# calderpg/voxelized_geometry_tools

Hardware: AMD Instinct MI355X
Metric: Mvoxels/s for 1024^3 float SDF extract @1 GPU; % HBM roofline (higher is better)
Workload: dtype int32; 1 GPU; 1024^3 float SDF, D1 spheres seed 42, res 0.01, device-resident; workload_key=c4, parallelism=single GPU, edt_variant=0

## Files before the change

include/vgt_hip.h:

```cpp
#ifndef VGT_HIP_H_
#define VGT_HIP_H_

#include <stddef.h>
#include <stdint.h>

#ifdef __cplusplus
extern "C" {
#endif
#if defined(__GNUC__) || defined(__clang__)
#pragma GCC visibility push(default)
#endif

#define VGT_HIP_ABI_VERSION 2

typedef struct vgt_hip_ctx vgt_hip_ctx;
typedef struct vgt_hip_grids vgt_hip_grids;
typedef struct vgt_hip_filter vgt_hip_filter;

enum {
  VGT_HIP_OK = 0,
  VGT_HIP_ERR_INVALID_ARGUMENT = 1,
  VGT_HIP_ERR_RUNTIME = 2,
  VGT_HIP_ERR_UNAVAILABLE = 3
};
// ... 27 lines not shown
                               float max_range, const float* grid_pointcloud_transform,
                               float voxel_size, float inverse_voxel_size,
                               float grid_x_size, float grid_y_size, float grid_z_size,
                               int32_t num_x_voxels, int32_t num_y_voxels,
                               int32_t num_z_voxels);
int vgt_hip_raycast_pointcloud2_f32(vgt_hip_ctx* ctx, vgt_hip_grids* grids, size_t grid_index,
                                    const uint8_t* cloud_data_host, int64_t num_points,
                                    int64_t point_step, int64_t xyz_offset, float max_range,
                                    const float* grid_pointcloud_transform, float voxel_size,
                                    float inverse_voxel_size, float grid_x_size,
                                    float grid_y_size, float grid_z_size, int32_t num_x_voxels,
                                    int32_t num_y_voxels, int32_t num_z_voxels);
int vgt_hip_raycast_points_f32_dev(vgt_hip_ctx* ctx, vgt_hip_grids* grids, size_t grid_index,
                                   const float* points_xyz_dev, int64_t num_points,
                                   float max_range, const float* grid_pointcloud_transform,
                                   float voxel_size, float inverse_voxel_size,
                                   float grid_x_size, float grid_y_size, float grid_z_size,
                                   int32_t num_x_voxels, int32_t num_y_voxels,
                                   int32_t num_z_voxels);
int vgt_hip_raycast_points_f64(vgt_hip_ctx* ctx, vgt_hip_grids* grids, size_t grid_index,
                               const double* points_xyz_host, int64_t num_points,
                               double max_range, const double* grid_pointcloud_transform,
                               double voxel_size, double inverse_voxel_size,
                               double grid_x_size, double grid_y_size, double grid_z_size,
                               int32_t num_x_voxels, int32_t num_y_voxels,
                               int32_t num_z_voxels);

int vgt_hip_filter_grid_create(vgt_hip_ctx* ctx, int64_t num_cells,
                               const float* occupancy_host, vgt_hip_filter** out_filter);
int vgt_hip_filter_grid_create_deferred(vgt_hip_ctx* ctx, int64_t num_cells,
                                        const float* occupancy_host, vgt_hip_filter** out_filter);
void vgt_hip_filter_grid_destroy(vgt_hip_filter* filter);
int64_t vgt_hip_filter_grid_num_cells(const vgt_hip_filter* filter);
void* vgt_hip_filter_grid_dev_ptr(const vgt_hip_filter* filter);

int vgt_hip_filter_tracking_grids(vgt_hip_ctx* ctx, const vgt_hip_grids* grids,
                                  float percent_seen_free, int32_t outlier_points_threshold,
                                  int32_t num_cameras_seen_free, vgt_hip_filter* filter);
int vgt_hip_filter_tracking_grids_f64(vgt_hip_ctx* ctx, const vgt_hip_grids* grids,
                                      double percent_seen_free,
                                      int32_t outlier_points_threshold,
                                      int32_t num_cameras_seen_free, vgt_hip_filter* filter);

int vgt_hip_retrieve_tracking_grid(vgt_hip_ctx* ctx, const vgt_hip_grids* grids,
                                   size_t grid_index, void* host_out);
int vgt_hip_retrieve_filtered_grid(vgt_hip_ctx* ctx, const vgt_hip_filter* filter,
                                   void* host_out);


int vgt_hip_sdf_from_occupancy_f32(vgt_hip_ctx* ctx, const float* occupancy_host,
                                   int64_t nx, int64_t ny, int64_t nz, double resolution,
                                   int unknown_is_filled, int add_virtual_border,
                                   float* sdf_host, float* out_min, float* out_max);
int vgt_hip_sdf_from_mask_u8(vgt_hip_ctx* ctx, const uint8_t* filled_mask_host, int64_t nx,
                             int64_t ny, int64_t nz, double resolution,
                             int add_virtual_border, float* sdf_host, float* out_min,
                             float* out_max);

size_t vgt_hip_sdf_workspace_bytes(int64_t nx, int64_t ny, int64_t nz);
size_t vgt_hip_sdf_workspace_bytes_for_variant(int64_t nx, int64_t ny, int64_t nz, int variant);
int vgt_hip_sdf_dev(vgt_hip_ctx* ctx, const float* occupancy_dev, int64_t nx, int64_t ny,
                    int64_t nz, double resolution, int unknown_is_filled,
                    int add_virtual_border, float* sdf_dev, void* workspace_dev,
                    size_t workspace_bytes, float* minmax_dev);
int vgt_hip_sdf_dev_timed(vgt_hip_ctx* ctx, const float* occupancy_dev, int64_t nx,
                          int64_t ny, int64_t nz, double resolution, int unknown_is_filled,
                          int add_virtual_border, float* sdf_dev, void* workspace_dev,
                          size_t workspace_bytes, float* minmax_dev, float* kernel_ms);
size_t vgt_hip_sdf_batch_workspace_bytes(int64_t batch, int64_t nx, int64_t ny, int64_t nz);
int vgt_hip_sdf_batch_dev(vgt_hip_ctx* ctx, const float* occupancy_dev, int64_t batch, int64_t nx, int64_t ny,
                          int64_t nz, double resolution, int unknown_is_filled, int add_virtual_border,
                          float* sdf_dev, void* workspace_dev, size_t workspace_bytes, float* minmax_dev);
int vgt_hip_sdf_batch_from_occupancy_f32(vgt_hip_ctx* ctx, const float* const* occupancy_host, int64_t batch,
                                         int64_t nx, int64_t ny, int64_t nz, double resolution,
                                         int unknown_is_filled, int add_virtual_border, float* const* sdf_host,
                                         float* out_min, float* out_max);
#ifdef VGT_HIP_TESTING
int vgt_hip_set_edt_variant(vgt_hip_ctx* ctx, int variant);
int vgt_hip_debug_finalize_check(vgt_hip_ctx* ctx, int64_t first_d2, int64_t count,
                                 double resolution, uint64_t* mismatches,
                                 uint64_t* first_mismatch);
int vgt_hip_testing_set_host_pipeline_min_voxels(int64_t min_voxels);
int vgt_hip_testing_set_short_line_rows(int rows);
int vgt_hip_testing_set_check_spheres_workgroups(int workgroups);
int vgt_hip_testing_set_sphere_volume_workgroups(int workgroups);
int vgt_hip_testing_set_align_workgroups(int workgroups);
int vgt_hip_testing_set_kinematics_workgroups(int workgroups);
int vgt_hip_testing_set_motion_workgroups(int workgroups);
int vgt_hip_testing_set_cost_workgroups(int workgroups);
int vgt_hip_testing_motion_launch_geometry(int64_t num_links, int64_t num_spheres, int32_t* tile_samples,
                                           int32_t* table_in_lds);
int vgt_hip_testing_cost_launch_geometry(int64_t num_links, int64_t num_spheres, int gradient_form, int32_t* tile_samples,
                                         int32_t* passes, int32_t* table_in_lds, int32_t* links_in_lds);
int vgt_hip_testing_set_self_collision_workgroups(int workgroups);
int vgt_hip_testing_set_motion_self_workgroups(int workgroups);
int vgt_hip_testing_set_sphere_volume_counters(uint64_t* counters_dev);
size_t vgt_hip_testing_class_record_bytes(int64_t nx, int64_t ny, int64_t nz);
int vgt_hip_testing_class_records_dev(vgt_hip_ctx* ctx, const float* occupancy_dev, int64_t nx, int64_t ny, int64_t nz,
                                      int unknown_is_filled, int64_t z_offset, void* records_dev, void* summary_dev);
#endif

typedef struct vgt_hip_cells vgt_hip_cells;
int vgt_hip_cells_create(vgt_hip_ctx* ctx, const void* cells_host, int64_t nx, int64_t ny,
                         int64_t nz, int32_t cell_bytes, int32_t object_id_offset,
                         vgt_hip_cells** out_cells);
void vgt_hip_cells_destroy(vgt_hip_cells* cells);
int vgt_hip_cells_object_ids(vgt_hip_ctx* ctx, vgt_hip_cells* cells, uint32_t* ids_out,
                             int64_t capacity, int64_t* count);
int vgt_hip_cells_sdf(vgt_hip_ctx* ctx, vgt_hip_cells* cells, const uint32_t* objects_to_use,
                      int64_t num_objects, double resolution, int unknown_is_filled,
                      int add_virtual_border, float* sdf_host, float* out_min, float* out_max);
int vgt_hip_cells_object_sdfs(vgt_hip_ctx* ctx, vgt_hip_cells* cells, const uint32_t* object_ids,
                              int64_t num_objects, double resolution, int unknown_is_filled, int add_virtual_border,
                              float* const* sdf_host, float* out_min, float* out_max);
int vgt_hip_cells_free_and_named_objects_sdf(vgt_hip_ctx* ctx, vgt_hip_cells* cells,
                                             double resolution, int unknown_is_filled,
                                             int add_virtual_border, float* sdf_host,
                                             float* out_min, float* out_max);

int vgt_hip_timing_start(vgt_hip_ctx* ctx, int32_t max_calls);
int vgt_hip_timing_stop(vgt_hip_ctx* ctx, float* kernel_ms ,
                        int32_t* num_calls);

int vgt_hip_sdf_coarse_gradient(vgt_hip_ctx* ctx, const float* sdf_host, int64_t nx, int64_t ny,
                                int64_t nz, double resolution, int enable_edge_gradients,
                                const double* rotation, double* gradient_host,
                                uint8_t* has_value_host);
int vgt_hip_sdf_coarse_gradient_dev(vgt_hip_ctx* ctx, const float* sdf_dev, int64_t nx, int64_t ny,
                                    int64_t nz, double resolution, int enable_edge_gradients,
                                    const double* rotation, double* gradient_dev,
                                    uint8_t* has_value_dev);

int vgt_hip_sdf_estimate_distance(vgt_hip_ctx* ctx, const float* sdf_host, int64_t nx, int64_t ny, int64_t nz,
                                  double resolution, const double* grid_from_world, const double* query_xyz_host,
                                  int64_t num_queries, double* distance_host, uint8_t* has_value_host);
int vgt_hip_sdf_estimate_distance_dev(vgt_hip_ctx* ctx, const float* sdf_dev, int64_t nx, int64_t ny, int64_t nz,
                                      double resolution, const double* grid_from_world, const double* query_xyz_dev,
                                      int64_t num_queries, double* distance_dev, uint8_t* has_value_dev);
int vgt_hip_sdf_fine_gradient(vgt_hip_ctx* ctx, const float* sdf_host, int64_t nx, int64_t ny, int64_t nz,
                              double resolution, const double* grid_from_world, const double* query_xyz_host,
                              int64_t num_queries, double nominal_window_size, double* gradient_host,
                              uint8_t* has_value_host);

#define VGT_HIP_PROJECT_OK 0
#define VGT_HIP_PROJECT_OUTSIDE 1
#define VGT_HIP_PROJECT_FLAT_GRADIENT 2
#define VGT_HIP_PROJECT_LEFT_GRID 3
#define VGT_HIP_PROJECT_ITERATION_LIMIT 4
int vgt_hip_sdf_project_out_of_collision(vgt_hip_ctx* ctx, const float* sdf_host, int64_t nx, int64_t ny, int64_t nz,
                                         double resolution, const double* grid_from_world, const double* rotation,
                                         const double* query_xyz_host, int64_t num_queries, double minimum_distance,
                                         double stepsize_multiplier, int32_t max_iterations, double* position_host,
                                         uint8_t* has_value_host, uint8_t* status_host, int32_t* iterations_host);
int vgt_hip_sdf_project_out_of_collision_dev(vgt_hip_ctx* ctx, const float* sdf_dev, int64_t nx, int64_t ny, int64_t nz,
                                             double resolution, const double* grid_from_world, const double* rotation,
                                             const double* query_xyz_dev, int64_t num_queries, double minimum_distance,
                                             double stepsize_multiplier, int32_t max_iterations, double* position_dev,
                                             uint8_t* has_value_dev, uint8_t* status_dev, int32_t* iterations_dev);

#define VGT_HIP_SEGMENT_OCCUPANCY 0
#define VGT_HIP_SEGMENT_SDF_BELOW 1
#define VGT_HIP_SEGMENT_WALK_THROUGH 1u
#define VGT_HIP_SEGMENT_CLEAR 0
#define VGT_HIP_SEGMENT_HIT 1
#define VGT_HIP_SEGMENT_MISSED_GRID 2
#define VGT_HIP_SEGMENT_INVALID 3
// ... 414 lines not shown
```

voxelized_geometry_tools_amd/capi.py:

```python
import collections
import ctypes
import threading
import weakref
import os

import numpy as np

_HERE = os.path.dirname(os.path.abspath(__file__))
LIB_PATH = os.environ.get("VGT_HIP_LIB") or os.path.join(_HERE, "libvgt_hip.so")
TESTING_LIB_PATH = os.environ.get("VGT_HIP_TESTING_LIB") or os.path.join(_HERE, "libvgt_hip_testing.so")
_LIB = None

_i64 = ctypes.c_int64
_i32 = ctypes.c_int32
_f32 = ctypes.c_float
_f64 = ctypes.c_double
_p = ctypes.c_void_p
_sz = ctypes.c_size_t
_int = ctypes.c_int

SIGNATURES = {
    "vgt_hip_abi_version": (_int, []),
    "vgt_hip_last_error": (ctypes.c_char_p, []),
    "vgt_hip_device_count": (_int, [ctypes.POINTER(_int)]),
# ... 104 lines not shown
    "vgt_hip_check_motions_with_self_dev": (_int, [_p, _p, _i64, _i64, _i64, _f64, _p, _p, _p, _p, _i64, _p, _i64, _p, _p,
                                                   _p, _p, _i32, _i64, _p, _p, _f64, _f64, ctypes.c_uint32, _p, _p, _p,
                                                   _p, _p, _p, _p, _p, _p, _p, _p]),
    "vgt_hip_motion_self_tile_samples": (_i32, [_i64, _i64]),
    "vgt_hip_nearest_workspace_bytes": (ctypes.c_size_t, [_i64, _i64, _i64]),
    "vgt_hip_nearest_dev": (_int, [_p, _p, _i64, _i64, _i64, _int, _p, _p, _p, ctypes.c_size_t]),
    "vgt_hip_nearest_from_occupancy_f32": (_int, [_p, _p, _i64, _i64, _i64, _int, _p, _p]),
    "vgt_hip_nearest_from_mask_u8": (_int, [_p, _p, _i64, _i64, _i64, _p, _p]),
    "vgt_hip_cells_nearest": (_int, [_p, _p, _p, _i64, _int, _p, _p, _p]),
    "vgt_hip_sdf_local_extrema_map": (_int, [_p, _p, _i64, _i64, _i64, _f64, _p, _p]),
    "vgt_hip_sdf_local_extrema_map_dev": (_int, [_p, _p, _i64, _i64, _i64, _f64, _p, _p]),
    "vgt_hip_connected_components": (_int, [_p, _p, _i64, _i64, _i64, _p, _p]),
    "vgt_hip_connected_components_dev": (_int, [_p, _p, _i64, _i64, _i64, _p, _p]),
    "vgt_hip_cells_connected_components": (_int, [_p, _p, _int, _p, _p]),
    "vgt_hip_cells_spatial_segments": (_int, [_p, _p, _p, _f64, _p, _p]),
    "vgt_hip_cells_spatial_segments_dev": (_int, [_p, _p, _p, _f64, _p, _p]),
    "vgt_hip_cells_update_spatial_segments": (_int, [_p, _p, _f64, _f64, _int, _int, _p, _p, _p]),
    "vgt_hip_component_surface_mask": (_int, [_p, _p, _p, _i64, _i64, _i64, _int, _p]),
    "vgt_hip_component_surface_mask_dev": (_int, [_p, _p, _p, _i64, _i64, _i64, _int, _p]),
    "vgt_hip_select_cells": (_int, [_p, _p, _p, _i64, _i64, _i64, _int, _int, _f32, _p, _p, _p, _i64, _p]),
    "vgt_hip_select_cells_dev": (_int, [_p, _p, _p, _i64, _i64, _i64, _int, _int, _f32, _p, _p, _p, _i64, _p]),
    "vgt_hip_cells_select": (_int, [_p, _p, _p, _int, _int, _p, _p, _p, _int, _i64, _p]),
    "vgt_hip_extract_surface": (_int, [_p, _p, _i64, _i64, _i64, _f32, _int, _f64, _p, _p, _p, _i64, _p, _i64, _p, _p]),
    "vgt_hip_extract_surface_dev": (_int, [_p, _p, _i64, _i64, _i64, _f32, _int, _f64, _p, _p, _p, _i64, _p, _i64, _p,
                                           _p]),
    "vgt_hip_cells_extract_surface": (_int, [_p, _p, _f64, _p, _p, _p, _i64, _p, _i64, _p, _p]),
    "vgt_hip_travel_cost_workspace_bytes": (ctypes.c_size_t, [_i64, _i64, _i64]),
    "vgt_hip_travel_cost": (_int, [_p, _p, _i64, _i64, _i64, _i32, _int, _f64, _p, ctypes.c_uint32, _p, _p, _i64,
                                   ctypes.c_uint32, _p, _p, _p]),
    "vgt_hip_travel_cost_dev": (_int, [_p, _p, _i64, _i64, _i64, _i32, _int, _f64, _p, ctypes.c_uint32, _p, _p, _i64,
                                       ctypes.c_uint32, _p, _p, _p, _p, _sz]),
    "vgt_hip_cells_travel_cost": (_int, [_p, _p, _p, _i64, _int, _p, ctypes.c_uint32, _p, _p, _i64, ctypes.c_uint32, _p,
                                         _p, _p]),
    "vgt_hip_trace_paths": (_int, [_p, _p, _i64, _p, _i64, _i32, _p, _p, _p]),
    "vgt_hip_trace_paths_dev": (_int, [_p, _p, _i64, _p, _i64, _i32, _p, _p, _p]),
    "vgt_hip_component_topology_dev": (_int, [_p, _p, _p, _i64, _i64, _i64, _int, ctypes.c_uint32, _p]),
    "vgt_hip_component_topology": (_int, [_p, _p, _i64, _i64, _i64, _int, _p, _p, _p, ctypes.c_uint64]),
    "vgt_hip_cells_component_topology": (_int, [_p, _p, _int, _int, _p, _p, _p, ctypes.c_uint64]),
    "vgt_hip_rasterize_mesh": (_int, [_p, _p, _i64, _p, _i64, _p, _int, _i64, _i64, _i64, _f64, _p, _p, _int, _int]),
    "vgt_hip_rasterize_mesh_dev": (_int, [_p, _p, _i64, _p, _i64, _p, _int, _i64, _i64, _i64, _f64, _p, _p, _int, _int]),
    "vgt_hip_mesh_grid_for": (_int, [_p, _i64, _f64, _p, _p, _p, _p]),
    "vgt_hip_fill_enclosed": (_int, [_p, _p, _int, _i64, _i64, _i64, _int, _p]),
    "vgt_hip_fill_enclosed_dev": (_int, [_p, _p, _int, _i64, _i64, _i64, _int, _p]),
    "vgt_hipx_sdf_multi": (_int, [_p, _int, _p, _i64, _i64, _i64, _f64, _int, _int, _p, _p, _p]),
    "vgt_hipx_release": (None, []),
    "vgt_hipx_last_timing": (_int, [_p]),
    "vgt_hipx_point_share": (_int, [_i64, _i32, _i32, _p, _p]),
    "vgt_hipx_raycast_points_split": (_int, [_p, _p, _sz, _p, _int, _p, _i64, _f32, _p, _f32, _f32, _f32, _f32,
                                             _f32, _i32, _i32, _i32]),
    "vgt_hip_sdf_dev": (_int, [_p, _p, _i64, _i64, _i64, _f64, _int, _int, _p, _p, _sz, _p]),
    "vgt_hip_sdf_dev_timed": (_int, [_p, _p, _i64, _i64, _i64, _f64, _int, _int, _p, _p, _sz, _p, _p]),
    "vgt_hip_sdf_batch_workspace_bytes": (_sz, [_i64, _i64, _i64, _i64]),
    "vgt_hip_sdf_batch_dev": (_int, [_p, _p, _i64, _i64, _i64, _i64, _f64, _int, _int, _p, _p, _sz, _p]),
    "vgt_hip_sdf_batch_from_occupancy_f32": (_int, [_p, _p, _i64, _i64, _i64, _i64, _f64, _int, _int, _p, _p, _p]),
    "vgt_hip_cells_object_sdfs": (_int, [_p, _p, _p, _i64, _f64, _int, _int, _p, _p, _p]),
    "vgt_hip_cells_create": (_int, [_p, _p, ctypes.c_int64, ctypes.c_int64, ctypes.c_int64, ctypes.c_int32,
                                   ctypes.c_int32, _p]),
    "vgt_hip_cells_destroy": (None, [_p]),
    "vgt_hip_cells_object_ids": (_int, [_p, _p, _p, ctypes.c_int64, _p]),
    "vgt_hip_cells_sdf": (_int, [_p, _p, _p, ctypes.c_int64, ctypes.c_double, _int, _int, _p, _p, _p]),
    "vgt_hip_cells_free_and_named_objects_sdf": (_int, [_p, _p, ctypes.c_double, _int, _int, _p, _p, _p]),
    "vgt_hip_sdf_coarse_gradient": (_int, [_p, _p, ctypes.c_int64, ctypes.c_int64, ctypes.c_int64, ctypes.c_double,
                                          _int, _p, _p, _p]),
    "vgt_hip_sdf_coarse_gradient_dev": (_int, [_p, _p, ctypes.c_int64, ctypes.c_int64, ctypes.c_int64,
                                              ctypes.c_double, _int, _p, _p, _p]),
    "vgt_hip_sdf_slab_carries_dev": (_int, [_p, _p, ctypes.c_int32, ctypes.c_int32, ctypes.c_int64, ctypes.c_int64,
                                            ctypes.c_int64, _p]),
    "vgt_hip_timing_start": (_int, [_p, ctypes.c_int32]),
    "vgt_hip_timing_stop": (_int, [_p, _p, _p]),
    "vgt_hip_sdf_slab_summary_bytes": (_sz, [_i64, _i64]),
    "vgt_hip_sdf_slab_carries_bytes": (_sz, [_i64, _i64]),
    "vgt_hip_sdf_slab_range": (_int, [_i64, ctypes.c_int32, ctypes.c_int32, _p, _p]),
    "vgt_hip_sdf_slab_begin_dev": (_int, [_p, _p, _i64, _i64, _i64, _i64, _int, _p, _sz, _p, _p]),
    "vgt_hip_sdf_slab_finish_dev": (_int, [_p, _i64, _i64, _i64, _i64, _i64, _f64, _int, _p, _p, _p,
                                           _sz, _p, _p]),
}


TESTING_SIGNATURES = {
    "vgt_hip_set_edt_variant": (_int, [_p, _int]),
    "vgt_hip_debug_finalize_check": (_int, [_p, ctypes.c_int64, ctypes.c_int64, ctypes.c_double, _p, _p]),
    "vgt_hip_testing_set_host_pipeline_min_voxels": (_int, [ctypes.c_int64]),
    "vgt_hip_testing_set_short_line_rows": (_int, [_int]),
    "vgt_hip_testing_set_check_spheres_workgroups": (_int, [_int]),
    "vgt_hip_testing_set_sphere_volume_workgroups": (_int, [_int]),
    "vgt_hip_testing_set_align_workgroups": (_int, [_int]),
    "vgt_hip_testing_set_kinematics_workgroups": (_int, [_int]),
    "vgt_hip_testing_set_motion_workgroups": (_int, [_int]),
    "vgt_hip_testing_set_cost_workgroups": (_int, [_int]),
    "vgt_hip_testing_motion_launch_geometry": (_int, [_i64, _i64, _p, _p]),
    "vgt_hip_testing_cost_launch_geometry": (_int, [_i64, _i64, _int, _p, _p, _p, _p]),
    "vgt_hip_testing_set_self_collision_workgroups": (_int, [_int]),
    "vgt_hip_testing_set_motion_self_workgroups": (_int, [_int]),
    "vgt_hip_testing_set_sphere_volume_counters": (_int, [_p]),
    "vgt_hip_testing_class_record_bytes": (_sz, [_i64, _i64, _i64]),
    "vgt_hip_testing_class_records_dev": (_int, [_p, _p, _i64, _i64, _i64, _int, _i64, _p, _p]),
}


MESH_RULE_REFERENCE = 0
MESH_RULE_NEAREST = 1

PROJECT_OK = 0
PROJECT_OUTSIDE = 1
PROJECT_FLAT_GRADIENT = 2
PROJECT_LEFT_GRID = 3
PROJECT_ITERATION_LIMIT = 4

SEGMENT_OCCUPANCY = 0
SEGMENT_SDF_BELOW = 1
SEGMENT_WALK_THROUGH = 1
SEGMENT_CLEAR = 0
SEGMENT_HIT = 1
SEGMENT_MISSED_GRID = 2
SEGMENT_INVALID = 3

SPHERES_OUTSIDE_IS_COLLISION = 1
SPHERES_CLEAR = 0
SPHERES_COLLISION = 1
SPHERES_NO_VALUE = 2
SPHERES_KEEP = 1
JOINT_FIXED, JOINT_REVOLUTE, JOINT_PRISMATIC = 0, 1, 2
FK_NOT_COMPUTABLE = 1
FK_OUTSIDE_LIMITS = 2
IK_CONVERGED = 0
IK_ITERATION_LIMIT = 1
IK_DEGENERATE = 2
IK_NOT_COMPUTABLE = 3
MOTION_STOP_AT_COLLISION = 2
MOTION_CLEAR = 0
MOTION_COLLISION = 1
MOTION_NO_VALUE = 2
MOTION_INVALID = 3
SELF_NO_VALUE_IS_COLLISION = 1
SELF_CLEAR = 0
SELF_COLLISION = 1
SELF_NO_VALUE = 2
SELF_PAIRS_SKIP_ADJACENT = 1
MOTION_SELF_NO_VALUE_IS_COLLISION = 4
MOTION_CAUSE_ENVIRONMENT = 1
MOTION_CAUSE_SELF = 2
ALIGN_CONVERGED = 0
ALIGN_ITERATION_LIMIT = 1
ALIGN_DEGENERATE = 2
ALIGN_TOO_FEW = 3

SELECT_ALL = 0
SELECT_SURFACE_26 = 1
SELECT_COMPONENT_SURFACE = 2
CLASS_ABOVE = 0x01
CLASS_BELOW = 0x02
CLASS_EQUAL = 0x04
CLASS_UNORDERED = 0x08
CELL_MEMBER_NONE = 0
CELL_MEMBER_OBJECT_ID = 1
CELL_MEMBER_COMPONENT = 2
CELL_MEMBER_SPATIAL_SEGMENT = 3

COMPONENT_TOPOLOGY = np.dtype([(name, np.int32) for name in (
    "present", "num_holes", "num_voids", "num_surfaces", "m3", "m5", "m6", "num_surface_vertices")])


SegmentCasts = collections.namedtuple("SegmentCasts", "status hit_index hit_fraction cells_examined min_value min_index")


SphereChecks = collections.namedtuple(
# ... 1030 lines not shown
        if not isinstance(cells, np.ndarray) or cells.ndim != 3 or not cells.flags.c_contiguous or \
                not cells.flags.writeable:
            raise ValueError("cells must be a writeable C-contiguous (nx, ny, nz) array")
        count = _i64(0)
        check(self._lib.vgt_hip_fill_enclosed(self.handle, _ptr(cells), cells.dtype.itemsize, *cells.shape,
                                              int(bool(unknown_is_filled)), ctypes.byref(count)))
        return int(count.value)

    def fill_enclosed_dev(self, cells_ptr, cell_bytes, shape, unknown_is_filled=True, want_count=True):
        count = _i64(0)
        check(self._lib.vgt_hip_fill_enclosed_dev(self.handle, _ptr(cells_ptr), int(cell_bytes),
                                                  *[int(c) for c in shape], int(bool(unknown_is_filled)),
                                                  ctypes.byref(count) if want_count else None))
        return int(count.value) if want_count else None

    def mesh_sdf(self, vertices, triangles, resolution, rule=MESH_RULE_REFERENCE, unknown_is_filled=True,
                 add_virtual_border=False, with_occupancy=False, solid=False):
        import torch
        v = np.ascontiguousarray(vertices, dtype=np.float64).reshape(-1, 3)
        t = np.ascontiguousarray(triangles, dtype=np.int32).reshape(-1, 3)
        shape, origin = mesh_grid_for(v, resolution)
        wfg = np.eye(4)
        wfg[:3, 3] = origin
        gfw = np.eye(4)
        gfw[:3, 3] = -origin
        device = "cuda:%d" % self._lib.vgt_hip_device_of(self.handle)
        v_dev = torch.from_numpy(v).to(device)
        t_dev = torch.from_numpy(t).to(device)
        occ_dev = torch.zeros(shape, dtype=torch.float32, device=device)
        sdf_dev = torch.empty(shape, dtype=torch.float32, device=device)
        ws_bytes = sdf_workspace_bytes(shape)
        ws_dev = torch.empty(ws_bytes, dtype=torch.uint8, device=device)
        minmax_dev = torch.empty(2, dtype=torch.float32, device=device)
        torch.cuda.synchronize(device)
        self.rasterize_mesh_dev(v_dev.data_ptr(), len(v), t_dev.data_ptr(), len(t), occ_dev.data_ptr(), 4, shape,
                                resolution, wfg.T.reshape(16), gfw.T.reshape(16), True, rule)
        if solid:
            self.fill_enclosed_dev(occ_dev.data_ptr(), 4, shape, unknown_is_filled, want_count=False)
        self.sdf_dev(occ_dev.data_ptr(), shape, resolution, sdf_dev.data_ptr(), ws_dev.data_ptr(), ws_bytes,
                     minmax_dev.data_ptr(), unknown_is_filled, add_virtual_border)
        self.synchronize()
        lo, hi = (float(x) for x in minmax_dev.cpu().numpy())
        out = (sdf_dev.cpu().numpy(), lo, hi, origin)
        return out + (occ_dev.cpu().numpy(),) if with_occupancy else out

    def trim(self):
        check(self._lib.vgt_hip_trim(self.handle))

    def set_stream(self, stream_ptr):
        check(self._lib.vgt_hip_set_stream(self.handle, _ptr(stream_ptr) if stream_ptr else None))

    def reset_stream(self):
        check(self._lib.vgt_hip_reset_stream(self.handle))

    def synchronize(self):
        check(self._lib.vgt_hip_synchronize(self.handle))

    def timing_start(self, max_calls):
        self._timing_capacity = int(max_calls)
        check(self._lib.vgt_hip_timing_start(self.handle, int(max_calls)))

    def timing_stop(self):
        out = np.zeros((self._timing_capacity, 3), dtype=np.float32)
        n = ctypes.c_int32(0)
        check(self._lib.vgt_hip_timing_stop(self.handle, _ptr(out), ctypes.byref(n)))
        return out[:n.value].copy()

    def set_edt_variant(self, variant):
        if not self.testing:
            if int(variant) == 0:
                return
            raise VgtHipError("EDT variants other than 0 exist in libvgt_hip_testing.so only: Context(testing=True)")
        check(self._lib.vgt_hip_set_edt_variant(self.handle, int(variant)))

    def class_records(self, occ_ptr, shape, unknown_is_filled=True, z_offset=0, records_ptr=None, summary_ptr=None):
        nx, ny, nz = shape
        check(self._lib.vgt_hip_testing_class_records_dev(self.handle, _ptr(occ_ptr), nx, ny, nz,
                                                          int(bool(unknown_is_filled)), int(z_offset), _ptr(records_ptr),
                                                          _ptr(summary_ptr)))

    def set_short_line_rows(self, rows):
        check(self._lib.vgt_hip_testing_set_short_line_rows(int(rows)))

    def set_check_spheres_workgroups(self, workgroups):
        check(self._lib.vgt_hip_testing_set_check_spheres_workgroups(int(workgroups)))

    def set_sphere_volume_workgroups(self, workgroups):
        check(self._lib.vgt_hip_testing_set_sphere_volume_workgroups(int(workgroups)))

    def set_align_workgroups(self, workgroups):
        check(self._lib.vgt_hip_testing_set_align_workgroups(int(workgroups)))

    def set_kinematics_workgroups(self, workgroups):
        check(self._lib.vgt_hip_testing_set_kinematics_workgroups(int(workgroups)))

    def set_motion_workgroups(self, workgroups):
        check(self._lib.vgt_hip_testing_set_motion_workgroups(int(workgroups)))

    def set_cost_workgroups(self, workgroups):
        check(self._lib.vgt_hip_testing_set_cost_workgroups(int(workgroups)))

    def set_self_collision_workgroups(self, workgroups):
        check(self._lib.vgt_hip_testing_set_self_collision_workgroups(int(workgroups)))

    def set_motion_self_workgroups(self, workgroups):
        check(self._lib.vgt_hip_testing_set_motion_self_workgroups(int(workgroups)))

    def set_sphere_volume_counters(self, counters_ptr):
        check(self._lib.vgt_hip_testing_set_sphere_volume_counters(_ptr(counters_ptr)))

    def set_host_pipeline_min_voxels(self, min_voxels):
        check(self._lib.vgt_hip_testing_set_host_pipeline_min_voxels(int(min_voxels)))

    def debug_finalize_check(self, first_d2, count, resolution):
        bad = ctypes.c_uint64(0)
        first = ctypes.c_uint64(0)
        check(self._lib.vgt_hip_debug_finalize_check(self.handle, int(first_d2), int(count), float(resolution),
                                                     ctypes.byref(bad), ctypes.byref(first)))
        return int(bad.value), (None if first.value == 2 ** 64 - 1 else int(first.value))

    def sdf_coarse_gradient(self, sdf, resolution, enable_edge_gradients=False, rotation=None):
        field = np.ascontiguousarray(sdf, dtype=np.float32)
        nx, ny, nz = field.shape
        grad = np.empty((nx, ny, nz, 3), dtype=np.float64)
        has = np.empty((nx, ny, nz), dtype=np.uint8)
        rot = None if rotation is None else np.ascontiguousarray(rotation, dtype=np.float64).reshape(9)
        check(self._lib.vgt_hip_sdf_coarse_gradient(self.handle, _ptr(field), nx, ny, nz, float(resolution),
                                                    int(bool(enable_edge_gradients)), _ptr(rot), _ptr(grad),
                                                    _ptr(has)))
        return grad, has.astype(bool)

    def cells(self, records, shape, object_id_offset=4):
        return Cells(self, records, shape, object_id_offset)

    def sdf_from_occupancy(self, occupancy, resolution, unknown_is_filled=True,
                           add_virtual_border=False, out=None):
        occ = np.ascontiguousarray(occupancy, dtype=np.float32)
        if occ.ndim != 3:
            raise ValueError("occupancy must be (nx, ny, nz)")
        nx, ny, nz = occ.shape
        if out is None:
            out = np.empty(occ.shape, dtype=np.float32)
        elif out.shape != occ.shape or out.dtype != np.float32 or not out.flags.c_contiguous:
            raise ValueError("out must be a C-contiguous float32 array of the occupancy's shape")
        lo, hi = _f32(), _f32()
        check(self._lib.vgt_hip_sdf_from_occupancy_f32(
            self.handle, _ptr(occ), nx, ny, nz, float(resolution), int(bool(unknown_is_filled)),
            int(bool(add_virtual_border)), _ptr(out), ctypes.byref(lo), ctypes.byref(hi)))
        return out, lo.value, hi.value

    def sdf_batch_from_occupancy(self, grids, resolution, unknown_is_filled=True, add_virtual_border=False):
        grids = [np.ascontiguousarray(g, dtype=np.float32) for g in grids]
        if not grids or any(g.ndim != 3 or g.shape != grids[0].shape for g in grids):
            raise ValueError("a batch is a non-empty list of (nx, ny, nz) grids of one shape")
        nx, ny, nz = grids[0].shape
        outs = [np.empty(g.shape, dtype=np.float32) for g in grids]
        batch = len(grids)
        in_ptrs = (ctypes.c_void_p * batch)(*[g.ctypes.data for g in grids])
        out_ptrs = (ctypes.c_void_p * batch)(*[o.ctypes.data for o in outs])
        lo = np.zeros(batch, dtype=np.float32)
        hi = np.zeros(batch, dtype=np.float32)
        check(self._lib.vgt_hip_sdf_batch_from_occupancy_f32(
            self.handle, ctypes.cast(in_ptrs, ctypes.c_void_p), batch, nx, ny, nz, float(resolution),
            int(bool(unknown_is_filled)), int(bool(add_virtual_border)), ctypes.cast(out_ptrs, ctypes.c_void_p),
            _ptr(lo), _ptr(hi)))
        return outs, lo, hi
# ... 567 lines not shown
```

voxelized_geometry_tools_amd/csrc/edt_kernels.hip:

```cpp
#include "edt_device.hpp"

namespace vgt
{
namespace
{
__global__ __launch_bounds__(256) void SlabCarriesKernel(const SlabLineSummary* __restrict__ summaries,
                                                        int world, int rank, int64_t lines, int nz_global,
                                                        SlabLineCarry* __restrict__ carries)
{
  const int share = nz_global / world, extra = nz_global % world;
  for (int64_t line = static_cast<int64_t>(blockIdx.x) * blockDim.x + threadIdx.x; line < lines;
       line += static_cast<int64_t>(gridDim.x) * blockDim.x)
  {
    int prev_filled = -1, prev_free = -1, next_filled = -1, next_free = -1;
    for (int r = 0; r < rank; r++)
    {
      const uint16_t rec = summaries[static_cast<int64_t>(r) * lines + line].last;
      const int end = (r + 1) * share + min(r + 1, extra) - 1;
      const int other = (rec & kSlabNone) == kSlabNone ? -1 : static_cast<int>(rec & kSlabNone);
      const bool filled = (rec & kSlabFilledBit) != 0;
      prev_filled = max(prev_filled, filled ? end : other);
      prev_free = max(prev_free, filled ? other : end);
    }
    for (int r = world - 1; r > rank; r--)
    {
      const uint16_t rec = summaries[static_cast<int64_t>(r) * lines + line].first;
      const int begin = r * share + min(r, extra);
      const int other = (rec & kSlabNone) == kSlabNone ? -1 : static_cast<int>(rec & kSlabNone);
      const bool filled = (rec & kSlabFilledBit) != 0;
      const int first_filled = filled ? begin : other, first_free = filled ? other : begin;
      if (first_filled >= 0) next_filled = first_filled;
      if (first_free >= 0) next_free = first_free;
    }
    SlabLineCarry c;
    c.prev_filled = static_cast<int16_t>(prev_filled);
    c.next_filled = static_cast<int16_t>(next_filled);
    c.prev_free = static_cast<int16_t>(prev_free);
    c.next_free = static_cast<int16_t>(next_free);
    carries[line] = c;
  }
}

__global__ void InitMinMaxKernel(uint32_t* minmax_enc, int count)
{
  for (int i = static_cast<int>(threadIdx.x); i < count; i += static_cast<int>(blockDim.x))
  {
    minmax_enc[2 * i] = 0xffffffffu;
    minmax_enc[2 * i + 1] = 0u;
  }
}
__global__ void DecodeMinMaxKernel(const uint32_t* minmax_enc, float* out, int count)
{
  for (int i = static_cast<int>(threadIdx.x); i < 2 * count; i += static_cast<int>(blockDim.x))
    out[i] = DecodeOrdered(minmax_enc[i]);
}

int GridFor(int64_t work_items, int block)
{
  const int64_t blocks = (work_items + block - 1) / block;
  const int64_t cap = 256 * 32;
  return static_cast<int>(blocks < 1 ? 1 : (blocks > cap ? cap : blocks));
}
}

hipError_t LaunchSlabCarries(const SlabLineSummary* summaries, int world, int rank, int64_t lines, int64_t nz_global,
                             SlabLineCarry* carries, hipStream_t stream)
{
  hipLaunchKernelGGL(SlabCarriesKernel, dim3(GridFor(lines, 256)), dim3(256), 0, stream, summaries, world, rank,
                     lines, static_cast<int>(nz_global), carries);
  return hipGetLastError();
}

hipError_t LaunchPassXFinalize(const int32_t* in32, float* sdf, uint32_t* minmax_enc, SweepScratch scratch,
                               const SdfParams& p, hipStream_t stream)
{
  return LaunchPassXFinalizeRange(in32, sdf, minmax_enc, scratch, p, 0, -1, stream);
}

hipError_t LaunchPassXFinalizeRange(const int32_t* in32, float* sdf, uint32_t* minmax_enc, SweepScratch scratch,
                                    const SdfParams& p, int64_t outer_begin, int64_t outer_count, hipStream_t stream)
{
  if (p.nx <= ShortLineRows())
    return LaunchPassXShortFinalizeRange(in32, sdf, minmax_enc, p, outer_begin, outer_count, stream);
  return LaunchPassXSweepFinalizeRange(in32, sdf, minmax_enc, scratch, p, outer_begin, outer_count, stream);
}

hipError_t LaunchInitMinMax(uint32_t* minmax_enc, hipStream_t stream, int64_t count)
{
  hipLaunchKernelGGL(InitMinMaxKernel, dim3(1), dim3(count > 1 ? 64 : 1), 0, stream, minmax_enc, static_cast<int>(count));
  return hipGetLastError();
}

hipError_t LaunchDecodeMinMax(const uint32_t* minmax_enc, float* minmax_out, hipStream_t stream, int64_t count)
{
  hipLaunchKernelGGL(DecodeMinMaxKernel, dim3(1), dim3(count > 1 ? 64 : 1), 0, stream, minmax_enc, minmax_out,
                     static_cast<int>(count));
  return hipGetLastError();
}
}
```

voxelized_geometry_tools_amd/csrc/edt_line_geom.hpp:

```cpp
#pragma once

#include "vgt_internal.hpp"

namespace vgt
{
struct SweepGeom
{
  int n;
  int nz;
  int zsegs;
  int items;
  int outers;
  int groups;
  int nwords;
  int chunks;
  int64_t row_stride;
  int64_t outer_stride;
  int nx, ny;
  int pass_axis;
  double resolution;
  int add_virtual_border;
  int z_offset, nz_global;
  int outer_begin;
  int batch_outers;
  int64_t batch_skip;
};

inline SweepGeom SweepGeometry(const SdfParams& p, int axis, int64_t* outer_count)
{
  SweepGeom g{};
  g.nz = static_cast<int>(p.nz);
  g.nx = static_cast<int>(p.nx);
  g.ny = static_cast<int>(p.ny);
  g.pass_axis = axis;
  if (axis == 0)
  {
    g.n = static_cast<int>(p.nx);
    g.row_stride = p.ny * p.nz;
    g.outer_stride = p.nz;
    *outer_count = p.ny;
  }
  else
  {
    g.n = static_cast<int>(p.ny);
    g.row_stride = p.nz;
    g.outer_stride = p.ny * p.nz;
    *outer_count = p.nx;
  }
  g.resolution = p.resolution;
  g.add_virtual_border = p.add_virtual_border;
  g.z_offset = static_cast<int>(p.z_offset);
  g.nz_global = static_cast<int>(p.nz_global > 0 ? p.nz_global : p.nz);
  return g;
}
}
```

voxelized_geometry_tools_amd/csrc/edt_record_kernels.hip:

```cpp
#include "edt_device.hpp"

#ifndef VGT_REC_EXP
#define VGT_REC_EXP 0
#endif
namespace vgt
{
namespace
{
constexpr int kRecordBlock = 256;
constexpr int kRecordWaves = kRecordBlock / kWaveSize;
constexpr int kNoTransitionBelow = -(1 << 20);
constexpr int kNoTransitionAbove = 1 << 20;

template <bool kUnknownFilled>
__device__ __forceinline__ bool IsFilledCell(float occupancy)
{
  return kUnknownFilled ? (occupancy >= 0.5f) : (occupancy > 0.5f);
}
template <bool kUnknownFilled>
__device__ __forceinline__ bool IsFilledCell(uint8_t mask)
{
  return mask != 0;
}

__device__ __forceinline__ void WriteLane(uint32_t& value, uint32_t word_uniform, int target)
{
  asm("s_nop 3\n\tv_writelane_b32 %0, %1, %2" : "+v"(value) : "s"(word_uniform), "n"(target));
}

__device__ __forceinline__ uint32_t EncodeBelow(int t, int word_begin)
{
  return (t == kNoTransitionBelow) ? kRecordNoneBelow : static_cast<uint32_t>(2 * (t - word_begin)) + kRecordBias;
}
__device__ __forceinline__ uint32_t EncodeAbove(int t, int word_begin)
{
  return (t == kNoTransitionAbove) ? kRecordNoneAbove : static_cast<uint32_t>(2 * (t - word_begin)) + kRecordBias;
}

__device__ __forceinline__ uint16_t SummaryField(bool filled, int other_local, int z_offset)
{
  return static_cast<uint16_t>((filled ? kSlabFilledBit : 0u) |
                               (other_local < 0 ? kSlabNone : static_cast<uint16_t>(other_local + z_offset)));
}

template <typename InT, int W, bool kUnknownFilled>
__global__ __launch_bounds__(kRecordBlock) void ClassRecordKernel(const InT* __restrict__ in,
                                                                 ClassRecord* __restrict__ records,
                                                                 int64_t num_lines, int ny, int nz, int nwords,
                                                                 SlabLineSummary* __restrict__ summary, int z_offset,
                                                                 int mark_no_site)
{
  constexpr int L = kWaveSize / W;
  const int lane = threadIdx.x & (kWaveSize - 1);
  const int wave = __builtin_amdgcn_readfirstlane(static_cast<int>(threadIdx.x) / kWaveSize);
  const int j = lane / W, w = lane % W;
  const int64_t num_steps = (num_lines + L - 1) / L;
  for (int64_t step = static_cast<int64_t>(blockIdx.x) * kRecordWaves + wave; step < num_steps;
       step += static_cast<int64_t>(gridDim.x) * kRecordWaves)
  {
    const int64_t line0 = step * L;
    const int lines_here = static_cast<int>(min(static_cast<int64_t>(L), num_lines - line0));
    InT v[L][W];
#pragma unroll
    for (int jj = 0; jj < L; jj++)
    {
      const InT* line_in = in + (line0 + min(jj, lines_here - 1)) * nz;
#pragma unroll
      for (int c = 0; c < W; c++)
      {
        const int z = min(min(c, nwords - 1) * kWaveSize + lane, nz - 1);
#if VGT_REC_EXP & 2
        v[jj][c] = line_in[z];
#else
        v[jj][c] = __builtin_nontemporal_load(line_in + z);
#endif
      }
    }
    uint32_t mlo = 0, mhi = 0;
#pragma unroll
    for (int jj = 0; jj < L; jj++)
    {
#pragma unroll
      for (int c = 0; c < W; c++)
      {
        const uint64_t m = __builtin_amdgcn_ballot_w64(IsFilledCell<kUnknownFilled>(v[jj][c]));
        WriteLane(mlo, static_cast<uint32_t>(m), jj * W + c);
        WriteLane(mhi, static_cast<uint32_t>(m >> 32), jj * W + c);
      }
    }
    const bool valid = j < lines_here && w < nwords;
    const uint64_t m = (static_cast<uint64_t>(mhi) << 32) | mlo;
    const uint32_t next_bit0 = static_cast<uint32_t>(__shfl_down(static_cast<int>(mlo & 1u), 1, W));
    const bool boundary = valid && (w + 1 < nwords) && (((mhi >> 31) & 1u) != next_bit0);
    const uint64_t inner = (m ^ (m >> 1)) & 0x7fffffffffffffffull;
    const uint64_t transitions = valid ? (inner | (boundary ? 0x8000000000000000ull : 0ull)) : 0ull;
    const int word_begin = w * kWaveSize;
    int last_t = kNoTransitionBelow, first_t = kNoTransitionAbove;
    if (transitions)
    {
      last_t = word_begin + 63 - __clzll(static_cast<long long>(transitions));
      first_t = word_begin + __ffsll(static_cast<long long>(transitions)) - 1;
    }
    int upto = last_t;
    int from = first_t;
#pragma unroll
    for (int d = 1; d < W; d *= 2)
    {
      const int a = __shfl_up(upto, d, W);
      const int b = __shfl_down(from, d, W);
      if (w >= d) upto = max(upto, a);
      if (w + d < W) from = min(from, b);
    }
    int below = __shfl_up(upto, 1, W);
    if (w == 0) below = kNoTransitionBelow;
    int above = __shfl_down(from, 1, W);
    if (w == W - 1) above = kNoTransitionAbove;
    if (boundary) above = word_begin + 63;
    const int line_last = __shfl(upto, W - 1, W);
    const int line_first = __shfl(from, 0, W);
    if (valid)
    {
      const uint32_t line = static_cast<uint32_t>(line0) + static_cast<uint32_t>(j);
      const int64_t x = line / static_cast<uint32_t>(ny);
      const int y = static_cast<int>(line - static_cast<uint32_t>(x) * static_cast<uint32_t>(ny));
      ClassRecord r;
      r.mask_lo = mlo;
      r.mask_hi = mhi;
      r.below2 = EncodeBelow(below, word_begin);
      r.above2 = EncodeAbove(above, word_begin);
      if (mark_no_site && line_last == kNoTransitionBelow) r.above2 = kRecordNoSite;
      using Raw = uint32_t __attribute__((ext_vector_type(4)));
      Raw raw;
      raw.x = r.mask_lo;
      raw.y = r.mask_hi;
      raw.z = r.below2;
      raw.w = r.above2;
#if VGT_REC_EXP & 1
      if (raw.x == 0x12345u)
#endif
      *reinterpret_cast<Raw*>(records + ((x * nwords + w) * ny + y)) = raw;
    }
    if (summary)
    {
      const uint32_t first_class = static_cast<uint32_t>(__shfl(static_cast<int>(mlo & 1u), 0, W));
      const int last_word = nwords - 1;
      const int last_bit = (nz - 1) & 63;
      const uint32_t my_last = static_cast<uint32_t>((m >> last_bit) & 1ull);
      const uint32_t last_class = static_cast<uint32_t>(__shfl(static_cast<int>(my_last), last_word, W));
      if (j < lines_here && w == 0)
      {
        SlabLineSummary s;
        s.first = SummaryField(first_class != 0u, line_first == kNoTransitionAbove ? -1 : line_first + 1, z_offset);
        s.last = SummaryField(last_class != 0u, line_last == kNoTransitionBelow ? -1 : line_last, z_offset);
        summary[line0 + j] = s;
      }
    }
  }
}

template <typename InT, bool kUnknownFilled>
__global__ __launch_bounds__(kRecordBlock) void ClassRecordLongLineKernel(const InT* __restrict__ in,
                                                                         ClassRecord* __restrict__ records,
                                                                         int64_t num_lines, int ny, int nz, int nwords,
                                                                         SlabLineSummary* __restrict__ summary,
                                                                         int z_offset, int mark_no_site)
{
  constexpr int kMaxWords = static_cast<int>(kMaxExtent / kWaveSize);
  __shared__ uint64_t s_mask[kRecordWaves][kMaxWords];
  __shared__ int32_t s_below[kRecordWaves][kMaxWords];
  __shared__ int32_t s_above[kRecordWaves][kMaxWords];
  __shared__ int32_t s_line[kRecordWaves][2];
  const int lane = threadIdx.x & (kWaveSize - 1);
  const int wave = threadIdx.x / kWaveSize;
  volatile uint64_t* mask = s_mask[wave];
  volatile int32_t* below = s_below[wave];
  volatile int32_t* above = s_above[wave];
  volatile int32_t* ends = s_line[wave];
  for (int64_t line = static_cast<int64_t>(blockIdx.x) * kRecordWaves + wave; line < num_lines;
       line += static_cast<int64_t>(gridDim.x) * kRecordWaves)
  {
    for (int c = 0; c < nwords; c++)
    {
      const int z = min(c * kWaveSize + lane, nz - 1);
      const uint64_t m = __builtin_amdgcn_ballot_w64(IsFilledCell<kUnknownFilled>(in[line * nz + z]));
      if (lane == 0) mask[c] = m;
    }
    __builtin_amdgcn_wave_barrier();
    if (lane == 0)
    {
      int last = kNoTransitionBelow;
      for (int c = 0; c < nwords; c++)
      {
        below[c] = last;
        const uint64_t m = mask[c];
        uint64_t t = (m ^ (m >> 1)) & 0x7fffffffffffffffull;
        if (c + 1 < nwords && ((m >> 63) & 1ull) != (mask[c + 1] & 1ull)) t |= 0x8000000000000000ull;
        if (t) last = c * kWaveSize + 63 - __clzll(static_cast<long long>(t));
      }
      ends[1] = last;
      int first = kNoTransitionAbove;
      for (int c = nwords - 1; c >= 0; c--)
      {
        const uint64_t m = mask[c];
        const bool boundary = c + 1 < nwords && ((m >> 63) & 1ull) != (mask[c + 1] & 1ull);
        above[c] = boundary ? c * kWaveSize + 63 : first;
        uint64_t t = (m ^ (m >> 1)) & 0x7fffffffffffffffull;
        if (boundary) t |= 0x8000000000000000ull;
        if (t) first = c * kWaveSize + __ffsll(static_cast<long long>(t)) - 1;
      }
      ends[0] = first;
    }
    __builtin_amdgcn_wave_barrier();
    const int64_t x = line / ny;
    const int y = static_cast<int>(line - x * ny);
    const int line_first = ends[0], line_last = ends[1];
    for (int c = lane; c < nwords; c += kWaveSize)
    {
      const uint64_t m = mask[c];
      ClassRecord r;
      r.mask_lo = static_cast<uint32_t>(m);
      r.mask_hi = static_cast<uint32_t>(m >> 32);
      r.below2 = EncodeBelow(below[c], c * kWaveSize);
      r.above2 = EncodeAbove(above[c], c * kWaveSize);
      if (mark_no_site && line_last == kNoTransitionBelow) r.above2 = kRecordNoSite;
      records[(x * nwords + c) * ny + y] = r;
    }
    if (summary && lane == 0)
    {
      const bool first_class = (mask[0] & 1ull) != 0ull;
      const bool last_class = ((mask[nwords - 1] >> ((nz - 1) & 63)) & 1ull) != 0ull;
      SlabLineSummary s;
      s.first = SummaryField(first_class, line_first == kNoTransitionAbove ? -1 : line_first + 1, z_offset);
      s.last = SummaryField(last_class, line_last == kNoTransitionBelow ? -1 : line_last, z_offset);
      summary[line] = s;
    }
    __builtin_amdgcn_wave_barrier();
  }
}

__global__ __launch_bounds__(256) void SlabRecordFixupKernel(ClassRecord* __restrict__ records,
                                                            const SlabLineCarry* __restrict__ carries, int64_t nx,
                                                            int ny, int nwords, int z_offset)
{
  const int64_t total = nx * nwords * static_cast<int64_t>(ny);
  for (int64_t i = static_cast<int64_t>(blockIdx.x) * blockDim.x + threadIdx.x; i < total;
       i += static_cast<int64_t>(gridDim.x) * blockDim.x)
  {
    ClassRecord r = records[i];
    const bool none_below = r.below2 == kRecordNoneBelow, none_above = r.above2 == kRecordNoneAbove;
    if (!none_below && !none_above) continue;
    const int y = static_cast<int>(i % ny);
    const int64_t xw = i / ny;
    const int w = static_cast<int>(xw % nwords);
    const int64_t x = xw / nwords;
    const SlabLineCarry c = carries[x * ny + y];
    const int word_begin = w * kWaveSize;
    bool changed = false;
    if (none_below)
    {
      const bool filled = (r.mask_lo & 1u) != 0u;
      const int other = filled ? c.prev_free : c.prev_filled;
      if (other >= 0)
      {
        r.below2 = EncodeBelow(other - z_offset, word_begin);
        changed = true;
      }
    }
    if (none_above)
    {
      const bool filled = (r.mask_hi >> 31) != 0u;
      const int other = filled ? c.next_free : c.next_filled;
      if (other >= 0)
      {
        r.above2 = EncodeAbove(other - 1 - z_offset, word_begin);
        changed = true;
      }
    }
    const uint64_t m = (static_cast<uint64_t>(r.mask_hi) << 32) | r.mask_lo;
    const bool uniform = (m ^ (m >> 1)) << 1 == 0ull;
    if (r.below2 == kRecordNoneBelow && r.above2 == kRecordNoneAbove && uniform)
    {
      r.above2 = kRecordNoSite;
      changed = true;
    }
    if (changed) records[i] = r;
  }
}

int RecordGridFor(int64_t steps)
{
  const int64_t blocks = (steps + kRecordWaves - 1) / kRecordWaves;
  const int64_t cap = 256 * 32;
  return static_cast<int>(blocks < 1 ? 1 : (blocks > cap ? cap : blocks));
}

template <typename InT, bool kUnknownFilled>
hipError_t LaunchRecords(const InT* in, ClassRecord* records, const SdfParams& p, SlabLineSummary* summary,
                         hipStream_t stream)
{
  const int64_t lines = p.nx * p.ny;
  const int nz = static_cast<int>(p.nz), ny = static_cast<int>(p.ny);
  const int nwords = static_cast<int>(RecordWords(p.nz));
  const int z_offset = static_cast<int>(p.z_offset);
  const int mark_no_site = summary == nullptr ? 1 : 0;
#define VGT_RECORD_CASE(W)                                                                                          \
  hipLaunchKernelGGL((ClassRecordKernel<InT, W, kUnknownFilled>), dim3(RecordGridFor((lines + 64 / W - 1) / (64 / W))), \
                     dim3(kRecordBlock), 0, stream, in, records, lines, ny, nz, nwords, summary, z_offset,          \
                     mark_no_site)
  if (nwords <= 1)
    VGT_RECORD_CASE(1);
  else if (nwords <= 2)
    VGT_RECORD_CASE(2);
  else if (nwords <= 4)
    VGT_RECORD_CASE(4);
  else if (nwords <= 8)
    VGT_RECORD_CASE(8);
  else if (nwords <= 16)
    VGT_RECORD_CASE(16);
  else if (nwords <= 32)
    VGT_RECORD_CASE(32);
  else if (nwords <= 64)
    VGT_RECORD_CASE(64);
  else
    hipLaunchKernelGGL((ClassRecordLongLineKernel<InT, kUnknownFilled>), dim3(RecordGridFor(lines)), dim3(kRecordBlock),
                       0, stream, in, records, lines, ny, nz, nwords, summary, z_offset, mark_no_site);
#undef VGT_RECORD_CASE
  return hipGetLastError();
}
}

hipError_t LaunchClassRecordsFromOccupancy(const float* occupancy, ClassRecord* records, const SdfParams& p,
                                           SlabLineSummary* summary, hipStream_t stream)
{
  if (p.unknown_is_filled) return LaunchRecords<float, true>(occupancy, records, p, summary, stream);
  return LaunchRecords<float, false>(occupancy, records, p, summary, stream);
}

hipError_t LaunchClassRecordsFromMask(const uint8_t* mask, ClassRecord* records, const SdfParams& p,
                                      SlabLineSummary* summary, hipStream_t stream)
{
  return LaunchRecords<uint8_t, false>(mask, records, p, summary, stream);
}

hipError_t LaunchSlabRecordFixup(ClassRecord* records, const SlabLineCarry* carries, const SdfParams& p,
                                 hipStream_t stream)
{
  const int nwords = static_cast<int>(RecordWords(p.nz));
  const int64_t total = p.nx * nwords * p.ny;
  const int64_t blocks = (total + 255) / 256;
  const int grid = static_cast<int>(blocks < 1 ? 1 : (blocks > 256 * 32 ? 256 * 32 : blocks));
  hipLaunchKernelGGL(SlabRecordFixupKernel, dim3(grid), dim3(256), 0, stream, records, carries, p.nx,
                     static_cast<int>(p.ny), nwords, static_cast<int>(p.z_offset));
  return hipGetLastError();
}
}
```

voxelized_geometry_tools_amd/csrc/edt_sweep_kernels.hip:

```cpp
#include "edt_device.hpp"
#include "edt_line_geom.hpp"

#include <cstdlib>
#include <type_traits>

namespace vgt
{
namespace
{
#ifndef VGT_SWEEP_BAND
#define VGT_SWEEP_BAND 16
#endif
#ifndef VGT_SWEEP_RING
#define VGT_SWEEP_RING 32
#endif
#ifndef VGT_SWEEP_CHUNK
#define VGT_SWEEP_CHUNK 8
#endif
#ifndef VGT_SWEEP_WAVES
#define VGT_SWEEP_WAVES 4
#endif
#ifndef VGT_SWEEP_GROUP
#define VGT_SWEEP_GROUP 2
#endif
constexpr int kBand = VGT_SWEEP_BAND;
constexpr int kWord = 32;
#ifndef VGT_SWEEP_INFO_BLOCK
#define VGT_SWEEP_INFO_BLOCK 2
#endif
constexpr int kInfoBlock = VGT_SWEEP_INFO_BLOCK;
static_assert(kInfoBlock >= 1, "sizes");
#ifndef VGT_SWEEP_RING_WIDE
#define VGT_SWEEP_RING_WIDE 16
#endif
#ifndef VGT_SWEEP_CHUNK_WIDE
#define VGT_SWEEP_CHUNK_WIDE 4
#endif
#ifndef VGT_SWEEP_GROUPS
#define VGT_SWEEP_GROUPS 8
#endif
constexpr int kSweepGroups = VGT_SWEEP_GROUPS;
constexpr int kCounterStride = 32;
constexpr int kMaxSweepSlots = 4096;
template <bool kPacked>
struct RingShape
{
  static constexpr int kRing = kPacked ? VGT_SWEEP_RING : VGT_SWEEP_RING_WIDE;
  static constexpr int kChunk = kPacked ? VGT_SWEEP_CHUNK : VGT_SWEEP_CHUNK_WIDE;
  static_assert(kBand % kChunk == 0 && kRing >= 4 * kChunk && (kRing & (kRing - 1)) == 0 && kChunk % 4 == 0, "sizes");
};
constexpr int kFar = 32768;
static_assert(kWord % kBand == 0 && kBand % 2 == 0, "sizes");
#ifdef VGT_HOST_EMULATION
uint64_t class_band_tally[3] = {0, 0, 0};
uint64_t ring_checks = 0, ring_spills = 0;
constexpr uint32_t kInfoPoison = 0xdeadbeefu;
uint64_t sign_word_reads = 0;
#endif


template <bool kPacked>
struct Codec;
template <>
struct Codec<true>
{
  using Entry = uint32_t;
  static constexpr int32_t kSentinelG = (1 << 22) - 3;
  static __device__ __forceinline__ Entry Pack(int32_t G, int row)
  {
    return (static_cast<uint32_t>(G) << 10) | static_cast<uint32_t>(row);
  }
  static __device__ __forceinline__ int32_t G(Entry e) { return static_cast<int32_t>(e >> 10); }
  static __device__ __forceinline__ int Row(Entry e) { return static_cast<int>(e & 1023u); }
  static __device__ __forceinline__ Entry Unknown() { return ~0u; }
  static __device__ __forceinline__ bool IsUnknown(Entry e) { return e == ~0u; }
};
template <>
struct Codec<false>
{
  using Entry = uint2;
  static constexpr int32_t kSentinelG = 1 << 30;
  static __device__ __forceinline__ Entry Pack(int32_t G, int row)
  {
    return make_uint2(static_cast<uint32_t>(G), static_cast<uint32_t>(row));
  }
  static __device__ __forceinline__ int32_t G(Entry e) { return static_cast<int32_t>(e.x); }
  static __device__ __forceinline__ int Row(Entry e) { return static_cast<int>(e.y); }
  static __device__ __forceinline__ Entry Unknown() { return make_uint2(0u, ~0u); }
  static __device__ __forceinline__ bool IsUnknown(Entry e) { return e.y == ~0u; }
};

#ifndef VGT_SWEEP_NT
#define VGT_SWEEP_NT 3
#endif
__device__ __forceinline__ void StoreQuad(uint4* p, uint32_t a, uint32_t b, uint32_t c, uint32_t d)
{
#if defined(VGT_HOST_EMULATION) || !(VGT_SWEEP_NT & 8)
  *p = make_uint4(a, b, c, d);
#else
  using Raw = uint32_t __attribute__((ext_vector_type(4)));
  Raw r;
  r.x = a; r.y = b; r.z = c; r.w = d;
  __builtin_nontemporal_store(r, reinterpret_cast<Raw*>(p));
#endif
}
__device__ __forceinline__ uint4 LoadQuad(const uint4* p)
{
#if defined(VGT_HOST_EMULATION) || !(VGT_SWEEP_NT & 8)
  return *p;
#else
  using Raw = uint32_t __attribute__((ext_vector_type(4)));
  const Raw r = __builtin_nontemporal_load(reinterpret_cast<const Raw*>(p));
  return make_uint4(r.x, r.y, r.z, r.w);
#endif
}
__device__ __forceinline__ void StorePair(uint2* p, uint32_t a, uint32_t b)
{
#if defined(VGT_HOST_EMULATION) || !(VGT_SWEEP_NT & 4)
  *p = make_uint2(a, b);
#else
  using Raw = uint32_t __attribute__((ext_vector_type(2)));
  Raw r;
  r.x = a; r.y = b;
  __builtin_nontemporal_store(r, reinterpret_cast<Raw*>(p));
#endif
}
__device__ __forceinline__ uint2 LoadPair(const uint2* p)
{
#if defined(VGT_HOST_EMULATION) || !(VGT_SWEEP_NT & 4)
  return *p;
#else
  using Raw = uint32_t __attribute__((ext_vector_type(2)));
  const Raw r = __builtin_nontemporal_load(reinterpret_cast<const Raw*>(p));
  return make_uint2(r.x, r.y);
#endif
}

template <int N>
__device__ __forceinline__ void StoreChunk(uint32_t* dst, const uint32_t (&e)[N])
{
// ... 109 lines not shown
__device__ __forceinline__ uint32_t AbsDiffPlusOne(uint32_t a, uint32_t b_uniform)
{
  return (max(a, b_uniform) - min(a, b_uniform)) + 1u;
}
__device__ __forceinline__ uint32_t SpreadLaneMask(uint64_t mask_uniform, [[maybe_unused]] int lane)
{
#ifdef VGT_HOST_EMULATION
  return ((mask_uniform >> lane) & 1ull) ? ~0u : 0u;
#else
  return __builtin_amdgcn_inverse_ballot_w64(mask_uniform) ? ~0u : 0u;
#endif
}

__device__ __forceinline__ void TakeLoaded([[maybe_unused]] uint32_t& v)
{
#ifndef VGT_HOST_EMULATION
  asm volatile("" : "+v"(v));
#endif
}
__device__ __forceinline__ void TakeLoaded(uint4& v)
{
  TakeLoaded(v.x);
  TakeLoaded(v.y);
  TakeLoaded(v.z);
  TakeLoaded(v.w);
}

__device__ __forceinline__ uint32_t LowBits(int bits)
{
  return (bits >= 32) ? ~0u : ((1u << bits) - 1u);
}

#if defined(VGT_HOST_EMULATION) || !(VGT_SWEEP_NT & 1)
#define VGT_STREAM_LOAD(p) (*(p))
#else
#define VGT_STREAM_LOAD(p) __builtin_nontemporal_load(p)
#endif
#if defined(VGT_HOST_EMULATION) || !(VGT_SWEEP_NT & 2)
#define VGT_STREAM_STORE(v, p) (*(p) = (v))
#else
#define VGT_STREAM_STORE(v, p) __builtin_nontemporal_store(v, p)
#endif

#ifdef VGT_HOST_EMULATION
#define VGT_COLD_PATH()
#define VGT_MIN_F32(acc, v) acc = fminf(acc, v)
#define VGT_MAX_F32(acc, v) acc = fmaxf(acc, v)
#define VGT_MIN3_F32(acc, a, b) acc = fminf(acc, fminf(a, b))
#define VGT_MAX3_F32(acc, a, b) acc = fmaxf(acc, fmaxf(a, b))
#else
#define VGT_COLD_PATH() asm volatile("; rare path")
#define VGT_MIN_F32(acc, v) asm("v_min_f32 %0, %0, %1" : "+v"(acc) : "v"(v))
#define VGT_MAX_F32(acc, v) asm("v_max_f32 %0, %0, %1" : "+v"(acc) : "v"(v))
#define VGT_MIN3_F32(acc, a, b) asm("v_min3_f32 %0, %0, %1, %2" : "+v"(acc) : "v"(a), "v"(b))
#define VGT_MAX3_F32(acc, a, b) asm("v_max3_f32 %0, %0, %1, %2" : "+v"(acc) : "v"(a), "v"(b))
#endif


__device__ __forceinline__ void WaveMinMax(float lo_value, float hi_value, uint32_t* minmax_enc)
{
  uint32_t lo = 0xffffffffu, hi = 0u;
  if (lo_value <= hi_value)
  {
    lo = EncodeOrdered(lo_value);
    hi = EncodeOrdered(hi_value);
  }
#ifdef VGT_HOST_EMULATION
  minmax_enc[0] = min(minmax_enc[0], lo);
  minmax_enc[1] = max(minmax_enc[1], hi);
#else
  for (int off = kWaveSize / 2; off > 0; off >>= 1)
  {
    lo = min(lo, static_cast<uint32_t>(__shfl_xor(static_cast<int>(lo), off)));
    hi = max(hi, static_cast<uint32_t>(__shfl_xor(static_cast<int>(hi), off)));
  }
  if (threadIdx.x == 0)
  {
    atomicMin(&minmax_enc[0], lo);
    atomicMax(&minmax_enc[1], hi);
  }
#endif
}

template <typename InT, typename OutT, bool kFinal, bool kPacked, bool kPlain>
__global__ __launch_bounds__(kWaveSize, VGT_SWEEP_WAVES) void SweepPassKernel(const InT* __restrict__ in,
                                                                            OutT* __restrict__ out,
                                                                            unsigned char* __restrict__ spill,
                                                                            uint2* __restrict__ word_info,
                                                                            uint32_t* __restrict__ minmax_enc,
                                                                            int* __restrict__ work_counter,
                                                                            const SweepGeom g)
{
  using C = Codec<kPacked>;
  using Entry = typename C::Entry;
  constexpr bool kRecords = std::is_same<InT, ClassRecord>::value;
  constexpr bool kSignBlocks = !kFinal;
  constexpr bool kTakeSignWords = !kSignBlocks;
  static_assert(!(kRecords && kFinal), "records feed the Y pass");
  constexpr int kRing = RingShape<kPacked>::kRing;
  constexpr int kChunk = RingShape<kPacked>::kChunk;
  constexpr int32_t kLimit = C::kSentinelG;
  constexpr int kEntryBytes = static_cast<int>(sizeof(Entry));
  constexpr int kShift = kPacked ? 8 : 9;
  constexpr uint32_t kSlot = 1u << kShift;
  constexpr uint32_t kRingMask = (kRing - 1) << kShift;
  constexpr int kChunkBytes = kChunk * kEntryBytes;
  constexpr uint32_t kChunkSlots = static_cast<uint32_t>(kChunk) << kShift;
  __shared__ Entry ring[kRing * kWaveSize];
  unsigned char* const ring_bytes = reinterpret_cast<unsigned char*>(ring);

  const int lane = threadIdx.x;
  const int n = g.n;
  const int64_t rstride = g.row_stride;
  unsigned char* const own_spill = spill + static_cast<int64_t>(blockIdx.x) * g.chunks * (kWaveSize * kChunkBytes);
  uint2* const own_info = word_info + static_cast<int64_t>(blockIdx.x) * (g.nwords + 1) * kWaveSize;
  const uint32_t lane_entry = static_cast<uint32_t>(lane) * kEntryBytes;
  const uint32_t lane_chunk = static_cast<uint32_t>(lane) * kChunkBytes;
  float lo_value = INFINITY, hi_value = -INFINITY;
  constexpr bool kUseTable = kFinal && kPlain && kPacked && (1024 / kBand <= 64);
  constexpr uint32_t kSmallD2 = 512;
  [[maybe_unused]] float* small_table = nullptr;
  if constexpr (kUseTable)
  {
    __shared__ float small_table_storage[kSmallD2];
    small_table = small_table_storage;
#ifdef VGT_HOST_EMULATION
    for (uint32_t d2 = 0; d2 < kSmallD2; d2++)
#else
    for (uint32_t d2 = static_cast<uint32_t>(lane); d2 < kSmallD2; d2 += kWaveSize)
#endif
      small_table[d2] = SqrtTimesResolutionExact(static_cast<int32_t>(d2), g.resolution);
    __syncthreads();
  }
#ifdef VGT_HOST_EMULATION
  int emulated_round = 0;
#endif
  [[maybe_unused]] auto fetch_item = [&]() -> int {
    int fetched = 0;
#ifndef VGT_HOST_EMULATION
    const int group = static_cast<int>(blockIdx.x) % g.groups;
    if (lane == 0) fetched = atomicAdd(work_counter + group * kCounterStride, 1);
    fetched = __builtin_amdgcn_readfirstlane(fetched);
    const int dealt = fetched / g.zsegs;
    fetched = (dealt * g.groups + group) * g.zsegs + (fetched - dealt * g.zsegs);
#endif
    return fetched;
  };
  for (;;)
  {
  int item = 0;
  unsigned char* wave_spill = own_spill;
  uint2* wave_info = own_info;
#ifdef VGT_HOST_EMULATION
  item = static_cast<int>(blockIdx.x + gridDim.x * emulated_round++);
#else
  item = fetch_item();
#endif
  if (item >= g.items) break;
#ifdef VGT_HOST_EMULATION
  for (int64_t w = 0; w < g.nwords + 1; w++) wave_info[w * kWaveSize + lane] = make_uint2(kInfoPoison, kInfoPoison);
#endif
  const int outer = item / g.zsegs;
  const int z0 = (item - outer * g.zsegs) * kWaveSize;
  const bool batched = g.batch_outers != g.outers;
  const int batch_index = batched ? outer / g.batch_outers : 0;
  const int outer_in_grid = outer - batch_index * g.batch_outers;
  const int64_t outer_offset = static_cast<int64_t>(outer) * g.outer_stride + static_cast<int64_t>(batch_index) * g.batch_skip;
  const uint32_t zl = static_cast<uint32_t>(min(lane, g.nz - 1 - z0));
  [[maybe_unused]] uint32_t lane_bytes = zl * 4u;
  const InT* const wave_in = kRecords ? in + static_cast<int64_t>(item) * n : in + (outer_offset + z0);
  OutT* const wave_out = out + (outer_offset + z0);

  uint32_t D = 4u << kShift, L = 0;
  int32_t Gt = C::kSentinelG, nB = 1;
  int rt = 0, A = 0;
  Entry e3 = C::Pack(C::kSentinelG + 2, 0);
  auto ring_ref = [&](uint32_t scaled_index) -> Entry& {
    return *reinterpret_cast<Entry*>(ring_bytes + ((scaled_index & kRingMask) | lane_entry));
  };
  auto chunk_in_ring = [&](uint32_t scaled_first) -> Entry* {
    return reinterpret_cast<Entry*>(ring_bytes + ((scaled_first & kRingMask) | lane_entry));
  };
  auto chunk_slot = [&](Entry* slots, uint32_t scaled_first, int j) -> Entry& {
    if constexpr (kPacked)
      return slots[j * kWaveSize];
    else
      return ring_ref(scaled_first + (static_cast<uint32_t>(j) << kShift));
  };
  static_assert(kRing % kChunk == 0, "a chunk must not wrap inside the ring");
  auto spill_ptr = [&](uint32_t scaled_first) -> Entry* {
    return reinterpret_cast<Entry*>(wave_spill + (scaled_first + lane_chunk));
  };
  ring_ref(0u << kShift) = C::Pack(0, 0);
  ring_ref(1u << kShift) = C::Pack(C::kSentinelG + 2, 0);
  ring_ref(2u << kShift) = C::Pack(C::kSentinelG + 1, 0);
  ring_ref(3u << kShift) = C::Pack(C::kSentinelG, 0);

  Entry pf0[kChunk], pf1[kChunk];
  int pf_count = 0;
  auto refill_now = [&]() {
    L -= kChunkSlots;
    const Entry* src = spill_ptr(L);
    Entry* const slots = chunk_in_ring(L);
#pragma unroll 1
    for (int j = 0; j < kChunk; j += 2)
    {
      const Entry a = src[j], b = src[j + 1];
      chunk_slot(slots, L, j) = a;
      chunk_slot(slots, L, j + 1) = b;
    }
    pf_count = 0;
  };
  auto pop = [&](auto third_in_register) {
    Gt += nB;
    rt -= A;
    if constexpr (decltype(third_in_register)::value)
    {
#ifdef VGT_HOST_EMULATION
      assert(!C::IsUnknown(e3));
#endif
    }
    else
    {
#ifdef VGT_HOST_EMULATION
      assert(C::IsUnknown(e3));
#endif
      if (__builtin_expect(D - 3 * kSlot < L, 0)) refill_now();
      e3 = ring_ref(D - 3 * kSlot);
    }
    A = rt - C::Row(e3);
    nB = C::G(e3) - Gt;
    D -= kSlot;
    e3 = C::Unknown();
  };
  auto commit = [&](const Entry (&buf)[kChunk]) {
    L -= kChunkSlots;
    Entry* const slots = chunk_in_ring(L);
#pragma unroll
    for (int j = 0; j < kChunk; j++) chunk_slot(slots, L, j) = buf[j];
  };

  uint32_t any_transition = 0;
  [[maybe_unused]] uint64_t small_bands = 0;
  {
    auto check_ring = [&]() {
      const uint32_t resident = D - L;
      const bool refilling = static_cast<int>(pf_count != 0) |
                             (static_cast<int>(L != 0) & static_cast<int>(resident <= kChunkSlots));
      if (__builtin_expect(__builtin_amdgcn_ballot_w64(refilling) != 0ull, 0))
      {
        VGT_COLD_PATH();
        if (pf_count != 0)
        {
          commit(pf0);
          pf_count = 0;
        }
        if (static_cast<int>(L != 0) & static_cast<int>(D - L <= kChunkSlots))
        {
          LoadChunk(spill_ptr(L - kChunkSlots), pf0);
          pf_count = 1;
        }
      }
      if (D - L > (static_cast<uint32_t>(kRing - kChunk) << kShift))
      {
        Entry buf[kChunk];
        Entry* const slots = chunk_in_ring(L);
#pragma unroll
        for (int j = 0; j < kChunk; j++) buf[j] = chunk_slot(slots, L, j);
        StoreChunk(spill_ptr(L), buf);
        L += kChunkSlots;
#ifdef VGT_HOST_EMULATION
        ring_spills++;
#endif
      }
#ifdef VGT_HOST_EMULATION
      ring_checks++;
      assert(D - L <= (static_cast<uint32_t>(kRing - kChunk) << kShift));
#endif
    };

    int din = kFar;
    uint32_t prev_bit = 0;
    uint32_t sw = 0;
    const int32_t n2m = 2 * (n - 1);
    auto site = [&](int q, int32_t G, bool wanted) {
      int32_t dG = G - Gt;
      int dr = q - rt;
      if (static_cast<int>(wanted) & static_cast<int>(dG < static_cast<int32_t>(__umul24(n2m, dr))))
      {
        if (static_cast<int64_t>(dG) * A + static_cast<int64_t>(nB) * dr < 0)
        {
          pop(std::true_type{});
          dG = G - Gt;
          dr = q - rt;
          if (__builtin_expect(static_cast<int64_t>(dG) * A + static_cast<int64_t>(nB) * dr < 0, 0))
          {
            do
            {
              pop(std::false_type{});
              dG = G - Gt;
              dr = q - rt;
            } while (static_cast<int64_t>(dG) * A + static_cast<int64_t>(nB) * dr < 0);
          }
        }
        ring_ref(D) = C::Pack(G, q);
        e3 = C::Pack(Gt + nB, rt - A);
        A = dr;
        nB = -dG;
        Gt = G;
        rt = q;
        D += kSlot;
      }
#ifndef VGT_HOST_EMULATION
      asm volatile("" : "+v"(Gt));
#endif
    };
    auto band_done = [&](int r0, uint32_t bits) {
      const int sub = r0 & (kWord - 1);
      sw |= (bits >> (32 - kBand)) << sub;
      if (sub + kBand == kWord || r0 + kBand >= n)
      {
        const int word_first = r0 - sub;
        const int valid = min(kWord, n - word_first);
        uint32_t xdn = sw ^ ((sw << 1) | prev_bit);
        xdn &= LowBits(valid);
        if (word_first == 0) xdn &= ~1u;
        StorePair(wave_info + static_cast<int64_t>(word_first / kWord) * kWaveSize + lane, sw, static_cast<uint32_t>(din));
        any_transition |= xdn;
        din = xdn ? (valid - (31 - __clz(static_cast<int>(xdn)))) : min(din + valid, kFar);
        prev_bit = (sw >> (valid - 1)) & 1u;
        sw = 0;
      }
// ... 69 lines not shown
        site(q, __mul24(f, f) + q * q, f2 < 2u * static_cast<uint32_t>(kInf16));
      };
      uint4 blk0 = load_block(0), blk1 = load_block(kBlock), blk2 = load_block(2 * kBlock);
      TakeLoaded(blk0);
      uint64_t marks = 0, filled = 0;
      constexpr uint32_t kBandMask = kBand >= 32 ? ~0u : ((1u << (kBand % 32)) - 1u);
      for (int r0 = 0; r0 < n; r0 += kBand)
      {
        __builtin_assume(r0 >= 0 && r0 < 16384);
        const int in_block = r0 & (kBlock - 1);
        const int block_first = r0 - in_block;
        if (in_block == 0) block_marks(blk0, r0, marks, filled);
        const uint32_t band_marks = static_cast<uint32_t>(marks >> in_block) & kBandMask;
        const uint32_t band_filled = static_cast<uint32_t>(filled >> in_block) & kBandMask;
        uint32_t bits;
        if (band_marks == kBandMask && r0 + kBand <= n)
        {
          bits = band_filled << (32 - kBand);
        }
        else
        {
          bits = 0;
#pragma unroll
          for (int k0 = 0; k0 < kBand; k0 += kRows)
          {
            const int q0 = r0 + k0;
            if (k0 % kChunk == 0) check_ring();
            if (((band_marks >> k0) & 0xfu) == 0xfu && q0 + kRows <= n)
              bits = __builtin_amdgcn_alignbit((band_filled >> k0) & 0xfu, bits, kRows);
            else
            {
#pragma unroll
              for (int k = 0; k < kRows; k++)
              {
                if (q0 + k < n)
                  row(q0 + k, record_of(blk0, block_first, in_block + k0 + k), bits);
                else
                  bits >>= 1;
              }
            }
          }
        }
        int moves_up = static_cast<int>(in_block + kBand == kBlock && r0 + kBand < n);
        if (moves_up)
        {
          blk0 = blk1;
          blk1 = blk2;
          TakeLoaded(blk0);
          TakeLoaded(blk1);
        }
#ifndef VGT_HOST_EMULATION
        asm volatile("" : "+v"(moves_up));
        moves_up = __builtin_amdgcn_readfirstlane(moves_up);
#endif
        if (moves_up) blk2 = load_block(r0 + kBand + 2 * kBlock);
        band_done(r0, bits);
      }
    }
    else
    {
      static_assert(kRecords || kFinal, "the X pass reads the Y pass's field");
      auto load_band = [&](int32_t (&dst)[kBand], int first_row) {
        const VGT_GLOBAL InT* row_in = UniformPointer(GlobalPointer(wave_in + static_cast<int64_t>(first_row) * rstride));
        if (first_row + kBand <= n)
        {
  #pragma unroll
          for (int k = 0; k < kBand; k++)
          {
            dst[k] = static_cast<int32_t>(VGT_STREAM_LOAD(LaneAddress(row_in, lane_bytes)));
            row_in = UniformPointer(row_in + rstride);
          }
        }
        else
        {
  #pragma unroll
          for (int k = 0; k < kBand; k++)
          {
            dst[k] = static_cast<int32_t>(VGT_STREAM_LOAD(LaneAddress(row_in, lane_bytes)));
            if (first_row + k + 1 < n) row_in = UniformPointer(row_in + rstride);
          }
        }
      };
      int32_t nxt[kBand];
      load_band(nxt, 0);
      constexpr int32_t kNoSiteG = 0x60000000;
      auto decode = [&](int32_t v, int q, int32_t& G) {
        const int32_t f = static_cast<int32_t>(min(static_cast<uint32_t>(v) & 0x7fffffffu, static_cast<uint32_t>(kNoSiteG)));
        G = f + q * q;
      };
      int32_t G_prev = kNoSiteG, G_cur = 0;
      decode(nxt[0], 0, G_cur);
      for (int r0 = 0; r0 < n; r0 += kBand)
      {
        __builtin_assume(r0 >= 0 && r0 < 16384);
        int32_t cur[kBand];
#pragma unroll
        for (int k = 0; k < kBand; k++) cur[k] = nxt[k];
        if (r0 + kBand < n) load_band(nxt, r0 + kBand);
        if constexpr (kUseTable)
        {
          uint32_t any = 0u;
#pragma unroll
          for (int k = 0; k < kBand; k++) any |= static_cast<uint32_t>(cur[k]);
          if (r0 + kBand <= n && __builtin_amdgcn_ballot_w64((any & 0x7fffffffu) >= kSmallD2) == 0ull)
            small_bands |= 1ull << (r0 / kBand);
        }
        uint32_t bits = 0;
        auto rows = [&](auto guarded) {
          constexpr bool kGuard = decltype(guarded)::value;
#pragma unroll
          for (int k = 0; k < kBand; k++)
          {
            if (k % kChunk == 0) check_ring();
            if (kGuard && r0 + k >= n) bits <<= 1;
            if (!kGuard || r0 + k < n)
            {
              const int q = r0 + k;
              bits = __builtin_amdgcn_alignbit(bits, static_cast<uint32_t>(cur[k]), 31);
              int32_t G_next = kNoSiteG + (q + 1) * (q + 1);
              if ((!kGuard && k + 1 < kBand) || q + 1 < n) decode(k + 1 < kBand ? cur[k + 1] : nxt[0], q + 1, G_next);
              site(q, G_cur, G_cur - G_prev < G_next - G_cur);
              G_prev = G_cur;
              G_cur = G_next;
            }
          }
        };
        if (r0 + kBand <= n)
          rows(std::false_type{});
        else
          rows(std::true_type{});
        band_done(r0, __builtin_bitreverse32(bits));
      }
    }
  }

  const bool classes = __builtin_amdgcn_ballot_w64(any_transition != 0u) != 0ull;
  const bool any_empty = __builtin_amdgcn_ballot_w64(D == (4u << kShift)) != 0ull;
  bool all_empty = !classes && __builtin_amdgcn_ballot_w64(D != (4u << kShift)) == 0ull;
  if constexpr (kFinal && !kPlain) all_empty = all_empty && !g.add_virtual_border;
  if (all_empty)
  {
    const int nwords = g.nwords;
    VGT_GLOBAL OutT* row_out = UniformPointer(GlobalPointer(wave_out + static_cast<int64_t>(n - 1) * rstride));
    uint2 info = LoadPair(wave_info + static_cast<int64_t>(nwords - 1) * kWaveSize + lane);
    for (int w = nwords - 1; w >= 0; w--)
    {
      const uint32_t sw = info.x;
#ifdef VGT_HOST_EMULATION
      assert(info.y != kInfoPoison);
      sign_word_reads++;
#endif
      if (w > 0) info = LoadPair(wave_info + static_cast<int64_t>(w - 1) * kWaveSize + lane);
      const int valid = min(kWord, n - w * kWord);
      if constexpr (kFinal)
      {
        const uint32_t rows_mask = LowBits(valid);
        if (sw & rows_mask) lo_value = -INFINITY;
        if (~sw & rows_mask) hi_value = INFINITY;
      }
      for (int k = valid - 1; k >= 0; k--)
      {
        const uint32_t sign = (sw >> k) << 31;
        if constexpr (kFinal)
        {
          VGT_STREAM_STORE(__uint_as_float(0x7f800000u | sign), LaneAddress(row_out, lane_bytes));
        }
        else
        {
          VGT_STREAM_STORE(static_cast<OutT>(static_cast<uint32_t>(kInf32) | sign), LaneAddress(row_out, lane_bytes));
        }
        row_out = UniformPointer(row_out - rstride);
      }
    }
  }
  else
  {
    pf_count = 0;
    auto refill_step = [&](auto commits, auto requests, Entry (&buf0)[kChunk], Entry (&buf1)[kChunk], int& count) {
      constexpr bool kCommits = decltype(commits)::value, kRequests = decltype(requests)::value;
      const bool refilling =
          (kCommits ? static_cast<int>(count != 0) : 0) |
          (kRequests ? (static_cast<int>(L != 0) & static_cast<int>(D - L <= (static_cast<uint32_t>(kRing - kChunk) << kShift))) : 0);
      if (__builtin_amdgcn_ballot_w64(refilling) != 0ull)
      {
        if constexpr (kCommits)
        {
          if (count > 0) commit(buf0);
          if (count > 1) commit(buf1);
          count = 0;
        }
        const uint32_t resident = D - L;
        if constexpr (kRequests)
        if (static_cast<int>(L != 0) & static_cast<int>(resident <= (static_cast<uint32_t>(kRing - kChunk) << kShift)))
        {
          LoadChunk(spill_ptr(L - kChunkSlots), buf0);
          count = 1;
          if (static_cast<int>(L != kChunkSlots) &
              static_cast<int>(resident <= (static_cast<uint32_t>(kRing - 2 * kChunk) << kShift)))
          {
            LoadChunk(spill_ptr(L - 2 * kChunkSlots), buf1);
            count = 2;
          }
        }
      }
// ... 308 lines not shown
          TakeLoaded(info_fresh.x);
          TakeLoaded(info_fresh.y);
          if (word_begins) info_next = info_fresh;
        }
      };
      bool small_band = false;
      if constexpr (kUseTable) small_band = ((small_bands >> (r0 / kBand)) & 1ull) != 0ull;
      bool without_candidates = false;
      if (classes && !any_empty && r0 + kBand <= n)
      {
        constexpr uint32_t kBandMask = kBand >= 32 ? ~0u : ((1u << (kBand % 32)) - 1u);
        const uint32_t touched = ((xdn_word | xup_word) >> sub) & kBandMask;
#ifdef VGT_HOST_EMULATION
        int ran = 2;
#endif
        if (__builtin_amdgcn_ballot_w64(touched != 0u) == 0ull)
        {
          const uint32_t below = xdn_word & LowBits(sub);
          const int d = below ? (sub - (31 - __clz(static_cast<int>(below)))) : static_cast<int>(info.y) + sub;
          const uint32_t delta = static_cast<uint32_t>(min(d, dn) + 1);
          __builtin_assume(rt >= 0 && rt < 16384);
          const int qt = r0 + kBand - 1;
          const int32_t p_first = Mad24Uniform(rt, -2 * r0, Gt) + r0 * r0;
          const int32_t p_last = Mad24Uniform(rt, -2 * qt, Gt) + qt * qt;
          const uint32_t B = static_cast<uint32_t>(max(p_first, p_last));
          const bool needed = static_cast<int>(B >= static_cast<uint32_t>(kLimit)) | static_cast<int>(B > delta * delta);
          without_candidates = __builtin_amdgcn_ballot_w64(needed) == 0ull;
          if (without_candidates) dn += kBand;
#ifdef VGT_HOST_EMULATION
          ran = without_candidates ? 1 : 0;
#endif
        }
#ifdef VGT_HOST_EMULATION
        if (any_transition != 0u) class_band_tally[ran]++;
#endif
      }
      const bool class_rows = classes && !without_candidates;
      if (r0 + kBand > n)
        rows(std::true_type{}, std::true_type{}, std::false_type{});
      else if (small_band)
      {
        if constexpr (kUseTable)
        {
          if (class_rows)
            rows(std::false_type{}, std::true_type{}, std::true_type{});
          else
            rows(std::false_type{}, std::false_type{}, std::true_type{});
        }
      }
      else if (class_rows || any_empty)
        rows(std::false_type{}, std::true_type{}, std::false_type{});
      else
        rows(std::false_type{}, std::false_type{}, std::false_type{});
      if (classes) dn = min(dn, kFar);
    }
  }
  if constexpr (kFinal)
  {
    if (batched)
    {
      WaveMinMax(lo_value, hi_value, minmax_enc + 2 * batch_index);
      lo_value = INFINITY;
      hi_value = -INFINITY;
    }
  }
  }
  if constexpr (kFinal) WaveMinMax(lo_value, hi_value, minmax_enc);
}

#ifdef VGT_HOST_EMULATION
constexpr int64_t kSweepSlots = 3;
#else
constexpr int64_t kSweepSlots = kMaxSweepSlots;
#endif
constexpr size_t kCounterBytes = (kSweepGroups * kCounterStride * sizeof(int) + 255) / 256 * 256;

int64_t SpillChunks(int64_t n, int chunk) { return (n + 4 + chunk - 1) / chunk + 1; }

bool PackedEntries(int64_t n, int64_t max_input)
{
  return n <= 1024 && max_input + (n - 1) * (n - 1) < Codec<true>::kSentinelG;
}

size_t SlotScratchBytes(int64_t n, bool packed)
{
  const int64_t nwords = (n + kWord - 1) / kWord;
  const size_t spill = packed ? SpillChunks(n, RingShape<true>::kChunk) * kWaveSize * RingShape<true>::kChunk * sizeof(uint32_t)
                              : SpillChunks(n, RingShape<false>::kChunk) * kWaveSize * RingShape<false>::kChunk * sizeof(uint2);
  return spill + static_cast<size_t>(nwords + 1) * kWaveSize * sizeof(uint2);
}

size_t PassScratchBytes(int64_t n, int64_t items, int64_t max_input)
{
  const int64_t slots = items < kSweepSlots ? items : kSweepSlots;
  const size_t planned = static_cast<size_t>(slots) * SlotScratchBytes(n, PackedEntries(n, max_input));
  const size_t one_wide = SlotScratchBytes(n, false);
  return kCounterBytes + (planned > one_wide ? planned : one_wide);
}

template <typename InT, typename OutT, bool kFinal>
hipError_t LaunchSweep(const InT* in, OutT* out, void* scratch, size_t scratch_bytes, uint32_t* minmax_enc, SweepGeom g,
                       int64_t outer_count, int64_t max_input, hipStream_t stream)
{
  g.zsegs = (g.nz + kWaveSize - 1) / kWaveSize;
  g.nwords = (g.n + kWord - 1) / kWord;
  const int64_t items = outer_count * g.zsegs;
  if (items <= 0) return hipSuccess;
  if (items > 0x7fffffffLL) return hipErrorInvalidValue;
  g.items = static_cast<int>(items);
  g.outers = static_cast<int>(outer_count);
  if (g.batch_outers <= 0)
  {
    g.batch_outers = g.outers;
    g.batch_skip = 0;
  }
  const bool packed = PackedEntries(g.n, max_input);
  int64_t slots = items < kSweepSlots ? items : kSweepSlots;
  {
    const size_t per_slot = SlotScratchBytes(g.n, packed);
    const int64_t fit = scratch_bytes > kCounterBytes ? static_cast<int64_t>((scratch_bytes - kCounterBytes) / per_slot) : 0;
    if (fit < 1) return hipErrorInvalidValue;
    if (fit < slots) slots = fit;
  }
  g.groups = static_cast<int>(slots < kSweepGroups ? slots : kSweepGroups);
  const int chunk = packed ? RingShape<true>::kChunk : RingShape<false>::kChunk;
  g.chunks = static_cast<int>(SpillChunks(g.n, chunk));
  char* bytes = static_cast<char*>(scratch);
  int* counter = reinterpret_cast<int*>(bytes);
  unsigned char* spill = reinterpret_cast<unsigned char*>(bytes + kCounterBytes);
  const size_t spill_bytes =
      static_cast<size_t>(slots) * g.chunks * kWaveSize * chunk * (packed ? sizeof(uint32_t) : sizeof(uint2));
  uint2* info = reinterpret_cast<uint2*>(bytes + kCounterBytes + spill_bytes);
#ifdef VGT_HOST_EMULATION
  *counter = 0;
#endif
  const dim3 grid(static_cast<unsigned>(slots)), block(kWaveSize);
  const bool general = kFinal && (g.add_virtual_border || !(g.resolution > 1.0e-30 && g.resolution < 1.0e30));
#ifndef VGT_HOST_EMULATION
  {
    const hipError_t err = hipMemsetAsync(counter, 0, kSweepGroups * kCounterStride * sizeof(int), stream);
    if (err != hipSuccess) return err;
  }
#endif
#define VGT_LAUNCH_SWEEP(PACKED, PLAIN)                                                                             \
  hipLaunchKernelGGL((SweepPassKernel<InT, OutT, kFinal, PACKED, PLAIN>), grid, block, 0, stream, in, out, spill, info, \
                     minmax_enc, counter, g)
  if (packed && general)
    VGT_LAUNCH_SWEEP(true, !kFinal);
  else if (packed)
    VGT_LAUNCH_SWEEP(true, true);
  else if (general)
    VGT_LAUNCH_SWEEP(false, !kFinal);
  else
    VGT_LAUNCH_SWEEP(false, true);
#undef VGT_LAUNCH_SWEEP
  return hipGetLastError();
}


int64_t MaxInputY(const SdfParams& p)
{
  const int64_t nzg = p.nz_global > 0 ? p.nz_global : p.nz;
  return (nzg - 1) * (nzg - 1);
}
int64_t MaxInputX(const SdfParams& p) { return MaxInputY(p) + (p.ny - 1) * (p.ny - 1); }
}

size_t SweepPassScratchBytes(int64_t nx, int64_t ny, int64_t nz, int64_t batch)
{
  const int64_t zsegs = (nz + kWaveSize - 1) / kWaveSize;
  const int64_t max_y = (nz - 1) * (nz - 1), max_x = max_y + (ny - 1) * (ny - 1);
  const size_t y = PassScratchBytes(ny, batch * nx * zsegs, max_y), x = PassScratchBytes(nx, batch * ny * zsegs, max_x);
  return (y > x ? y : x) + 256;
}

hipError_t LaunchPassYSweepRecords(const ClassRecord* records, int32_t* out32, SweepScratch scratch, const SdfParams& p,
                                   hipStream_t stream)
{
#ifndef VGT_HOST_EMULATION
  if (p.ny <= ShortLineLimit(p.nx * ((p.nz + kWaveSize - 1) / kWaveSize))) return LaunchPassYShortRecords(records, out32, p, stream);
#endif
  int64_t outer_count = 0;
  const SweepGeom g = SweepGeometry(p, 1, &outer_count);
  return LaunchSweep<ClassRecord, int32_t, false>(records, out32, scratch.ptr, scratch.bytes, nullptr, g, outer_count,
                                                  MaxInputY(p), stream);
}

hipError_t LaunchPassXSweepFinalizeRange(const int32_t* in32, float* sdf, uint32_t* minmax_enc, SweepScratch scratch,
                                         const SdfParams& p, int64_t outer_begin, int64_t outer_count_or_all,
                                         hipStream_t stream)
{
  int64_t outer_count = 0;
  SweepGeom g = SweepGeometry(p, 0, &outer_count);
  if (p.batch > 1)
  {
    if (outer_count_or_all >= 0 || p.batch * outer_count > 0x7fffffffLL) return hipErrorInvalidValue;
    g.batch_outers = static_cast<int>(outer_count);
    g.batch_skip = (p.nx - 1) * p.ny * p.nz;
    outer_count *= p.batch;
  }
  if (outer_count_or_all >= 0)
  {
    in32 += outer_begin * g.outer_stride;
    sdf += outer_begin * g.outer_stride;
    g.outer_begin = static_cast<int>(outer_begin);
    outer_count = outer_count_or_all;
  }
  return LaunchSweep<int32_t, float, true>(in32, sdf, scratch.ptr, scratch.bytes, minmax_enc, g, outer_count,
                                           MaxInputX(p), stream);
}

hipError_t LaunchPassXSweepFinalize(const int32_t* in32, float* sdf, uint32_t* minmax_enc, SweepScratch scratch,
                                    const SdfParams& p, hipStream_t stream)
{
  return LaunchPassXSweepFinalizeRange(in32, sdf, minmax_enc, scratch, p, 0, -1, stream);
}

}
```

voxelized_geometry_tools_amd/csrc/vgt_hip_capi.hip:

```cpp
#include "../../include/vgt_hip.h"

#include "vgt_internal.hpp"
#include "nearest_internal.hpp"
#include "device_memory.hpp"
#include "host_staging.hpp"
#include "mesh_kernels.hpp"
#include "edt_crosscheck.hpp"
#include "host_pages.hpp"

#include <algorithm>
#include <cmath>
#include <limits>
#include <atomic>
#include <cstdio>
#include <cstring>
#include <functional>
#include <map>
#include <memory>
#include <mutex>
#include <vector>
#include <new>
#include <string>
#include <thread>
#ifdef __linux__
// ... 24 lines not shown
  std::atomic<unsigned> next_lane{0};
  vgt::DeviceCache ray_scratch;
  vgt::DeviceCache minmax_out;
  int variant = 0;
  std::vector<hipEvent_t> timing_events;
  std::vector<uint8_t> timing_kind;
  int timing_slots = 0;
  int timing_used = 0;
  vgt::DeviceCache sdf_in, sdf_out, sdf_ws;
  vgt::DeviceCache component_ws;
  vgt::DeviceCache select_ws;
  vgt::DeviceCache surface_ws;
  vgt::DeviceCache mesh_ws;
  void* host_staging = nullptr;
  std::vector<hipEvent_t> staging_events;
  std::atomic<int> children{0};
  std::atomic<bool> destroyed{false};
  std::vector<vgt::DeviceCache> pool;
  size_t pool_bytes = 0;
  bool pool_closed = false;
  struct SlabNote
  {
    int64_t z_offset, nz_local, nz_global;
  };
  std::map<const void*, SlabNote> slab_notes;
  hipStream_t copy_in = nullptr;
  hipStream_t copy_out = nullptr;
  std::vector<hipEvent_t> pipeline_events;
};

struct vgt_hip_grids
{
  vgt_hip_ctx* ctx = nullptr;
  int device = -1;
  vgt::DeviceCache dev;
  int64_t num_cells = 0;
  int32_t num_grids = 0;
};

struct vgt_hip_filter
{
  vgt_hip_ctx* ctx = nullptr;
  int device = -1;
  vgt::DeviceCache dev;
  int64_t num_cells = 0;
  hipEvent_t uploaded = nullptr;
  bool upload_pending = false;
  void* pin = nullptr;
};

struct vgt_hip_kinematics
{
  vgt_hip_ctx* ctx = nullptr;
  int device = -1;
  int64_t num_links = 0, num_joints = 0;
  int lds_links = 0;
  vgt::DeviceTemp links;
  vgt::DeviceTemp limits;
  vgt::DeviceTemp chain;
  std::vector<vgt::KinematicLink> host_links;
};

struct vgt_hip_cells
{
  vgt_hip_ctx* ctx = nullptr;
  int device = -1;
  int64_t nx = 0, ny = 0, nz = 0;
  int cell_bytes = 0;
  int object_id_offset = -1;
  vgt::DeviceTemp records;
  vgt::DeviceTemp mask;
  vgt::DeviceTemp sdf;
  vgt::DeviceCache sdf_named;
  vgt::DeviceCache workspace;
  vgt::DeviceCache objects;
  vgt::DeviceTemp scalar;
  vgt::DeviceCache batch_masks, batch_sdf, batch_ws;
};

namespace
{
thread_local std::string g_last_error;
std::atomic<int> g_short_line_override{-1};
std::atomic<int> g_check_spheres_workgroups{0};
std::atomic<int> g_align_workgroups{0};
std::atomic<int> g_kinematics_workgroups{0};
std::atomic<int> g_motion_workgroups{0};
std::atomic<int> g_cost_workgroups{0};
std::atomic<int> g_self_collision_workgroups{0};
std::atomic<int> g_motion_self_workgroups{0};
std::atomic<int> g_sphere_volume_workgroups{0};
std::atomic<unsigned long long*> g_sphere_volume_counters{nullptr};

int Fail(int code, const std::string& msg)
{
  g_last_error = msg;
  return code;
}

}
namespace vgt
{
void SetLastError(const std::string& message) { g_last_error = message; }
hipStream_t ContextStream(const vgt_hip_ctx* ctx) { return ctx->stream; }
int ShortLineOverride() { return g_short_line_override.load(); }
}
namespace
{
int FailHip(const char* what, hipError_t err)
{
  g_last_error = std::string("[") + what + "] HIP error [" + hipGetErrorString(err) + "]";
  return VGT_HIP_ERR_RUNTIME;
}

void AdoptChild(vgt_hip_ctx* ctx) { ctx->children.fetch_add(1); }
void ReleaseChild(vgt_hip_ctx* ctx, int device)
{
  if (!ctx) return;
  (void)hipSetDevice(device);
  if (ctx->destroyed.load())
    (void)hipDeviceSynchronize();
  else
    (void)hipStreamSynchronize(ctx->stream);
  if (ctx->children.fetch_sub(1) == 1 && ctx->destroyed.load()) delete ctx;
}

#define VGT_TRY_HIP(expr, what)                          \
  do                                                     \
  {                                                      \
    const hipError_t vgt_err_ = (expr);                  \
    if (vgt_err_ != hipSuccess) return FailHip(what, vgt_err_); \
  } while (0)

int HipResult(const char* what, hipError_t err) { return err == hipSuccess ? VGT_HIP_OK : FailHip(what, err); }

size_t AlignUp(size_t v, size_t a) { return (v + a - 1) / a * a; }

constexpr size_t kPoolLimit = size_t{4} << 30;
hipError_t PoolAllocate(vgt_hip_ctx* ctx, vgt::DeviceCache* buffer, size_t bytes)
{
  {
    std::lock_guard<std::mutex> lock(ctx->mutex);
    for (size_t i = 0; i < ctx->pool.size(); i++)
      if (ctx->pool[i].bytes() == bytes)
      {
        *buffer = std::move(ctx->pool[i]);
        ctx->pool_bytes -= bytes;
        ctx->pool.erase(ctx->pool.begin() + static_cast<std::ptrdiff_t>(i));
        return hipSuccess;
      }
  }
  return buffer->Reserve(bytes);
}
void PoolRelease(vgt_hip_ctx* ctx, vgt::DeviceCache* buffer)
{
  if (!buffer->data()) return;
  if (ctx && !ctx->destroyed.load())
  {
    std::lock_guard<std::mutex> lock(ctx->mutex);
    if (!ctx->pool_closed && ctx->pool_bytes + buffer->bytes() <= kPoolLimit && ctx->pool.size() < 16)
    {
      ctx->pool_bytes += buffer->bytes();
      ctx->pool.push_back(std::move(*buffer));
      return;
    }
  }
  (void)buffer->Release();
}
void FreePool(vgt_hip_ctx* ctx)
{
  ctx->pool.clear();
  ctx->pool_bytes = 0;
}

hipError_t DrainKeepingFirst(hipStream_t s, hipError_t err)
{
  const hipError_t sync = hipStreamSynchronize(s);
  return err == hipSuccess ? sync : err;
}

template <typename T>
hipError_t ReadBack(hipStream_t s, hipError_t launched, T* value, const void* value_dev)
{
  if (launched == hipSuccess) launched = hipMemcpyAsync(value, value_dev, sizeof(T), hipMemcpyDeviceToHost, s);
  return DrainKeepingFirst(s, launched);
}

int GrowCache(hipStream_t s, vgt::DeviceCache* cache, size_t need, const char* drain_what, const char* allocate_what,
// ... 74 lines not shown
  }
  static std::map<const void*, Entry>& Table()
  {
    static auto* table = new std::map<const void*, Entry>();
    return *table;
  }
  const void* shared_ = nullptr;
};

#ifdef VGT_HIP_TESTING
constexpr bool kHaveCrossCheck = true;
#else
constexpr bool kHaveCrossCheck = false;
#endif

struct SdfWorkspace
{
  vgt::ClassRecord* records;
  int16_t* t16;
  int32_t* t32;
  uint32_t* minmax_enc;
  vgt::SweepScratch sweep_scratch;
  size_t bytes;
};

SdfWorkspace CarveWorkspace(void* base, int64_t nx, int64_t ny, int64_t nz, int variant, int64_t batch = 1)
{
  SdfWorkspace ws;
  const size_t n = static_cast<size_t>(batch * nx * ny * nz);
  size_t off = 0;
  ws.records = nullptr;
  ws.t16 = nullptr;
  if (kHaveCrossCheck && variant != 0)
  {
    ws.t16 = reinterpret_cast<int16_t*>(static_cast<char*>(base) + off);
    off = AlignUp(off + vgt::CrossCheckFieldBytes(batch * nx * ny * nz), 256);
  }
  else
  {
    ws.records = reinterpret_cast<vgt::ClassRecord*>(static_cast<char*>(base) + off);
    off = AlignUp(off + vgt::ClassRecordBytes(batch * nx, ny, nz), 256);
  }
  ws.t32 = reinterpret_cast<int32_t*>(static_cast<char*>(base) + off);
  off = AlignUp(off + n * sizeof(int32_t), 256);
  ws.minmax_enc = reinterpret_cast<uint32_t*>(static_cast<char*>(base) + off);
  off += AlignUp(static_cast<size_t>(batch) * 2 * sizeof(uint32_t), 256);
  ws.sweep_scratch.ptr = static_cast<char*>(base) + off;
  ws.sweep_scratch.bytes = vgt::SweepPassScratchBytes(nx, ny, nz, batch);
  off = AlignUp(off + ws.sweep_scratch.bytes, 256);
  ws.bytes = off;
  return ws;
}

template <typename InT>
hipError_t LaunchPassOne(const InT* input_dev, const SdfWorkspace& ws, const vgt::SdfParams& part, int64_t first_slice,
                         vgt::SlabLineSummary* summary, hipStream_t s)
{
  const int64_t voxel_offset = first_slice * part.ny * part.nz;
  if constexpr (kHaveCrossCheck)
  {
    if (ws.t16)
    {
      if constexpr (std::is_same<InT, float>::value)
        return vgt::LaunchCrossCheckScanZFromOccupancy(input_dev + voxel_offset, ws.t16 + voxel_offset, part, summary, s);
      else
        return vgt::LaunchCrossCheckScanZFromMask(input_dev + voxel_offset, ws.t16 + voxel_offset, part, summary, s);
    }
  }
  vgt::ClassRecord* records = ws.records + first_slice * vgt::RecordWords(part.nz) * part.ny;
  if constexpr (std::is_same<InT, float>::value)
    return vgt::LaunchClassRecordsFromOccupancy(input_dev + voxel_offset, records, part, summary, s);
  else
    return vgt::LaunchClassRecordsFromMask(input_dev + voxel_offset, records, part, summary, s);
}
hipError_t LaunchPassTwo(const SdfWorkspace& ws, const vgt::SdfParams& part, int64_t first_slice, hipStream_t s)
{
  const int64_t voxel_offset = first_slice * part.ny * part.nz;
  if constexpr (kHaveCrossCheck)
  {
    if (ws.t16) return vgt::LaunchCrossCheckPassY(ws.t16 + voxel_offset, ws.t32 + voxel_offset, part, s);
  }
  return vgt::LaunchPassYSweepRecords(ws.records + first_slice * vgt::RecordWords(part.nz) * part.ny,
                                      ws.t32 + voxel_offset, ws.sweep_scratch, part, s);
}
hipError_t LaunchPassThree(const SdfWorkspace& ws, const vgt::SdfParams& p, float* sdf_dev, hipStream_t s)
{
  if constexpr (kHaveCrossCheck)
  {
    if (ws.t16) return vgt::LaunchCrossCheckPassXFinalize(ws.t32, sdf_dev, ws.minmax_enc, p, s);
  }
  return vgt::LaunchPassXFinalize(ws.t32, sdf_dev, ws.minmax_enc, ws.sweep_scratch, p, s);
}
hipError_t LaunchSlabFixup(const SdfWorkspace& ws, const vgt::SlabLineCarry* carries, const vgt::SdfParams& p, hipStream_t s)
{
  if constexpr (kHaveCrossCheck)
  {
    if (ws.t16) return vgt::LaunchCrossCheckSlabFixup(ws.t16, carries, p, s);
  }
  return vgt::LaunchSlabRecordFixup(ws.records, carries, p, s);
}

int CheckSdfShape(int64_t nx, int64_t ny, int64_t nz, double resolution)
{
  if (nx <= 0 || ny <= 0 || nz <= 0)
    return Fail(VGT_HIP_ERR_INVALID_ARGUMENT, "grid extents must be positive");
  if (nx > vgt::kMaxExtent || ny > vgt::kMaxExtent || nz > vgt::kMaxExtent)
    return Fail(VGT_HIP_ERR_INVALID_ARGUMENT, "grid extent exceeds 16384 voxels on an axis");
  if (!(resolution > 0.0) || !std::isfinite(resolution))
    return Fail(VGT_HIP_ERR_INVALID_ARGUMENT, "Grid must have uniform, positive resolution");
  return VGT_HIP_OK;
}

int CheckProjectionArguments(int64_t nx, int64_t ny, int64_t nz, double resolution, double minimum_distance,
                             double stepsize_multiplier, int32_t max_iterations)
{
  const int rc = CheckSdfShape(nx, ny, nz, resolution);
  if (rc != VGT_HIP_OK) return rc;
  if (nx * ny * nz >= 0x7fffffffLL)
    return Fail(VGT_HIP_ERR_INVALID_ARGUMENT, "the projection out of collision supports grids below 2^31 cells");
  if (std::isnan(minimum_distance)) return Fail(VGT_HIP_ERR_INVALID_ARGUMENT, "minimum_distance must not be NaN");
  if (!(stepsize_multiplier > 0.0) || !std::isfinite(stepsize_multiplier))
    return Fail(VGT_HIP_ERR_INVALID_ARGUMENT, "stepsize_multiplier must be positive and finite");
  if (max_iterations < 0) return Fail(VGT_HIP_ERR_INVALID_ARGUMENT, "max_iterations must not be negative");
  return VGT_HIP_OK;
}

int CheckSegmentArguments(const vgt_hip_ctx* ctx, const float* field, int64_t nx, int64_t ny, int64_t nz,
                          double resolution, int32_t mode, int unknown_is_filled, double threshold, uint32_t flags,
                          const double* grid_from_world, const double* segments, int64_t num_segments,
                          const uint8_t* status, const float* min_value, const int32_t* min_index,
                          vgt::SegmentGrid* grid, vgt::SegmentQuery* query)
{
  if (!ctx || !field || !status || num_segments < 0 || (num_segments > 0 && !segments))
    return Fail(VGT_HIP_ERR_INVALID_ARGUMENT, "null argument");
  if (nx < 0 || ny < 0 || nz < 0) return Fail(VGT_HIP_ERR_INVALID_ARGUMENT, "grid extents must not be negative");
  if (!(resolution > 0.0) || !std::isfinite(resolution))
    return Fail(VGT_HIP_ERR_INVALID_ARGUMENT, "Grid must have uniform, positive resolution");
  const int64_t most = 0x7fffffffLL;
  if (nx > most || ny > most || nz > most || (nx > 0 && ny > 0 && nz > 0 && (nx * ny > most || nx * ny * nz > most)))
    return Fail(VGT_HIP_ERR_INVALID_ARGUMENT, "segment casts support grids below 2^31 cells");
  if (mode != VGT_HIP_SEGMENT_OCCUPANCY && mode != VGT_HIP_SEGMENT_SDF_BELOW)
    return Fail(VGT_HIP_ERR_INVALID_ARGUMENT, "unknown segment cast mode");
  if (flags & ~VGT_HIP_SEGMENT_WALK_THROUGH) return Fail(VGT_HIP_ERR_INVALID_ARGUMENT, "unknown segment cast flag");
  if (mode == VGT_HIP_SEGMENT_SDF_BELOW && std::isnan(threshold))
    return Fail(VGT_HIP_ERR_INVALID_ARGUMENT, "threshold must not be NaN");
  if (mode == VGT_HIP_SEGMENT_OCCUPANCY && (min_value || min_index))
    return Fail(VGT_HIP_ERR_INVALID_ARGUMENT, "min_value and min_index are outputs of the SDF mode");
  grid->has_xform = grid_from_world ? 1 : 0;
  for (int k = 0; k < 16; k++) grid->xform[k] = grid_from_world ? grid_from_world[k] : 0.0;
  grid->voxel_size = resolution;
  grid->inverse_voxel_size = 1.0 / resolution;
  const int64_t counts[3] = {nx, ny, nz};
  for (int a = 0; a < 3; a++)
  {
    grid->counts[a] = static_cast<int32_t>(counts[a]);
    grid->grid_size[a] = static_cast<double>(counts[a]) * resolution;
  }
  query->mode = mode == VGT_HIP_SEGMENT_OCCUPANCY ? vgt::kSegmentOccupancy : vgt::kSegmentSdfBelow;
  query->unknown_is_filled = unknown_is_filled ? 1 : 0;
  query->threshold = threshold;
  query->flags = flags;
  return VGT_HIP_OK;
}

struct AlignPointsArguments
{
// ... 172 lines not shown
                                  padding};
  }
};

struct RasterizeSpheresArguments
{
  int64_t nx, ny, nz;
  double resolution;
  const double* grid_from_world;
  SphereVolumeArguments body;
  int64_t base;
  uint32_t flags;
  int32_t* first_configuration;

  int64_t NumCells() const { return nx * ny * nz; }
  bool Keep() const { return (flags & VGT_HIP_SPHERES_KEEP) != 0; }
  int Check(const vgt_hip_ctx* ctx) const
  {
    int rc = body.CheckCounts();
    if (rc != VGT_HIP_OK) return rc;
    if (!ctx || !first_configuration || body.MissingModel()) return Fail(VGT_HIP_ERR_INVALID_ARGUMENT, "null argument");
    if (nx < 0 || ny < 0 || nz < 0) return Fail(VGT_HIP_ERR_INVALID_ARGUMENT, "grid extents must not be negative");
    if (!(resolution > 0.0) || !std::isfinite(resolution))
      return Fail(VGT_HIP_ERR_INVALID_ARGUMENT, "Grid must have uniform, positive resolution");
    const int64_t most = 0x7fffffffLL;
    if (nx > most || ny > most || nz > most || (nx > 0 && ny > 0 && nz > 0 && (nx * ny > most || nx * ny * nz > most)))
      return Fail(VGT_HIP_ERR_INVALID_ARGUMENT, "sphere volumes support grids below 2^31 cells");
    if (flags & ~VGT_HIP_SPHERES_KEEP) return Fail(VGT_HIP_ERR_INVALID_ARGUMENT, "unknown sphere-volume flag");
    rc = body.Check();
    if (rc != VGT_HIP_OK) return rc;
    if (base < 0 || base > most - body.num_configurations)
      return Fail(VGT_HIP_ERR_INVALID_ARGUMENT,
                  "first_configuration_base must not be negative, and base + configurations at most 2^31 - 1");
    return VGT_HIP_OK;
  }
  hipError_t Launch(const double* xyzr_dev, const int32_t* link_dev, const double* poses_dev, int32_t* first_dev,
                    hipStream_t stream) const
  {
    return vgt::LaunchRasterizeSpheres(nx, ny, nz, resolution, grid_from_world,
                                       body.Model(xyzr_dev, link_dev, poses_dev), base, Keep(), first_dev,
                                       g_sphere_volume_workgroups.load(), g_sphere_volume_counters.load(), stream);
  }
};

struct CoverPointsArguments
{
  const float* points;
  int64_t num_points;
  const double* world_from_points;
  SphereVolumeArguments body;
  uint32_t flags;
  int32_t *first_configuration, *first_sphere;
  float* filtered;

  int Check(const vgt_hip_ctx* ctx) const
  {
    int rc = body.CheckCounts();
    if (rc != VGT_HIP_OK) return rc;
    if (num_points < 0) return Fail(VGT_HIP_ERR_INVALID_ARGUMENT, "the number of points must not be negative");
    if (!ctx || (num_points > 0 && !points) || (!first_configuration && !first_sphere && !filtered) ||
        body.MissingModel())
      return Fail(VGT_HIP_ERR_INVALID_ARGUMENT, "null argument");
    if (num_points > 0x7fffffffLL) return Fail(VGT_HIP_ERR_INVALID_ARGUMENT, "sphere volumes support fewer than 2^31 points");
    if (flags) return Fail(VGT_HIP_ERR_INVALID_ARGUMENT, "unknown sphere-volume flag");
    return body.Check();
  }
  hipError_t Launch(const float* points_dev, const double* xyzr_dev, const int32_t* link_dev, const double* poses_dev,
                    int32_t* first_configuration_dev, int32_t* first_sphere_dev, float* filtered_dev,
                    hipStream_t stream) const
  {
    return vgt::LaunchCoverPoints(points_dev, num_points, world_from_points, body.Model(xyzr_dev, link_dev, poses_dev),
                                  first_configuration_dev, first_sphere_dev, filtered_dev,
                                  g_sphere_volume_workgroups.load(), stream);
  }
};

hipEvent_t* TimingSlot(vgt_hip_ctx* ctx)
{
  if (ctx->timing_slots == 0 || ctx->timing_used >= ctx->timing_slots) return nullptr;
  return &ctx->timing_events[static_cast<size_t>(ctx->timing_used) * 8];
}

template <typename InT>
int RunSdfPipeline(vgt_hip_ctx* ctx, const InT* input_dev, const vgt::SdfParams& p, float* sdf_dev,
                   void* workspace_dev, size_t workspace_bytes, float* minmax_dev,
                   hipEvent_t* events)
{
  if (p.batch > 1 && ctx->variant != 0)
    return Fail(VGT_HIP_ERR_INVALID_ARGUMENT, "batches run on the default EDT pipeline only");
  const SdfWorkspace ws = CarveWorkspace(workspace_dev, p.nx, p.ny, p.nz, ctx->variant, p.batch);
  if (workspace_dev == nullptr || workspace_bytes < ws.bytes)
    return Fail(VGT_HIP_ERR_INVALID_ARGUMENT, "SDF workspace too small");
  hipStream_t s = ctx->stream;
  vgt::SdfParams slices = p;
  slices.nx = p.nx * p.batch;
  slices.batch = 1;
  VGT_TRY_HIP(vgt::LaunchInitMinMax(ws.minmax_enc, s, p.batch), "init min/max");
  if (events) VGT_TRY_HIP(hipEventRecord(events[0], s), "event record");
  VGT_TRY_HIP(LaunchPassOne<InT>(input_dev, ws, slices, 0, nullptr, s), "pass 1");
  if (events) VGT_TRY_HIP(hipEventRecord(events[1], s), "event record");
  VGT_TRY_HIP(LaunchPassTwo(ws, slices, 0, s), "Y pass");
  if (events) VGT_TRY_HIP(hipEventRecord(events[2], s), "event record");
  VGT_TRY_HIP(LaunchPassThree(ws, p, sdf_dev, s), "X pass");
  if (events) VGT_TRY_HIP(hipEventRecord(events[3], s), "event record");
  if (minmax_dev) VGT_TRY_HIP(vgt::LaunchDecodeMinMax(ws.minmax_enc, minmax_dev, s, p.batch), "min/max");
  return VGT_HIP_OK;
}

int CheckBatch(int64_t batch, int64_t nx, int64_t ny, int64_t nz)
{
  if (batch <= 0) return Fail(VGT_HIP_ERR_INVALID_ARGUMENT, "batch must be positive");
  const int64_t zsegs = (nz + 63) / 64;
  if (batch > (int64_t{1} << 20) || batch * nx * ny >= (int64_t{1} << 28) || batch * nx * zsegs > 0x7fffffffLL ||
      batch * ny * zsegs > 0x7fffffffLL)
    return Fail(VGT_HIP_ERR_INVALID_ARGUMENT, "batch too large: batch * nx * ny must stay below 2^28 lines");
  return VGT_HIP_OK;
}

constexpr size_t kStagingSlotBytes = size_t{8} << 20;
constexpr int kStagingSlots = 4;
struct HostArrayCopy
{
  const void* device;
  void* host;
};
hipError_t EnsureStaging(vgt_hip_ctx* ctx)
{
  if (ctx->host_staging) return hipSuccess;
  const hipError_t err = hipHostMalloc(&ctx->host_staging, kStagingSlots * kStagingSlotBytes, hipHostMallocDefault);
  if (err != hipSuccess)
  {
    ctx->host_staging = nullptr;
    (void)hipGetLastError();
  }
  return err;
}
struct RingPiece
{
  size_t first, count;
  size_t offset;
  size_t bytes;
};
std::vector<RingPiece> RingPieces(const std::vector<HostArrayCopy>& arrays, size_t bytes)
{
  std::vector<RingPiece> pieces;
  if (bytes >= kStagingSlotBytes)
  {
    for (size_t a = 0; a < arrays.size(); a++)
      for (size_t off = 0; off < bytes; off += kStagingSlotBytes)
        pieces.push_back(RingPiece{a, 1, off, std::min(kStagingSlotBytes, bytes - off)});
    return pieces;
  }
  const size_t per_slot = kStagingSlotBytes / bytes;
  for (size_t a = 0; a < arrays.size();)
  {
    size_t count = 1;
    while (count < per_slot && a + count < arrays.size() &&
           static_cast<const char*>(arrays[a + count].device) == static_cast<const char*>(arrays[a].device) + count * bytes)
      count++;
    pieces.push_back(RingPiece{a, count, 0, count * bytes});
    a += count;
  }
  return pieces;
}
void CopyPieceRange(const std::vector<HostArrayCopy>& arrays, size_t bytes, const RingPiece& p, char* slot, size_t begin,
                    size_t end, bool to_host)
{
  while (begin < end)
  {
    const size_t k = p.count == 1 ? 0 : begin / bytes;
    const size_t in_array = p.count == 1 ? p.offset + begin : begin - k * bytes;
    const size_t array_end = p.count == 1 ? end : std::min(end, (k + 1) * bytes);
    char* const host = static_cast<char*>(arrays[p.first + k].host) + in_array;
    if (to_host)
      std::memcpy(host, slot + begin, array_end - begin);
    else
// ... 570 lines not shown
{
  if (!ctx) return Fail(VGT_HIP_ERR_INVALID_ARGUMENT, "null argument");
  {
    std::lock_guard<std::mutex> lock(ctx->mutex);
    VGT_TRY_HIP(hipSetDevice(ctx->device), "set device");
    VGT_TRY_HIP(hipStreamSynchronize(ctx->stream), "drain stream");
    FreeCachedSdfBuffers(ctx);
    FreePool(ctx);
  }
  FreeUploadLanes(ctx, false);
  return VGT_HIP_OK;
}

int vgt_hip_set_stream(vgt_hip_ctx* ctx, void* hip_stream)
{
  if (!ctx) return Fail(VGT_HIP_ERR_INVALID_ARGUMENT, "null argument");
  std::lock_guard<std::mutex> lock(ctx->mutex);
  VGT_TRY_HIP(hipSetDevice(ctx->device), "set device");
  VGT_TRY_HIP(hipStreamSynchronize(ctx->stream), "drain stream");
  ctx->stream = static_cast<hipStream_t>(hip_stream);
  return VGT_HIP_OK;
}

int vgt_hip_reset_stream(vgt_hip_ctx* ctx)
{
  if (!ctx) return Fail(VGT_HIP_ERR_INVALID_ARGUMENT, "null argument");
  std::lock_guard<std::mutex> lock(ctx->mutex);
  VGT_TRY_HIP(hipSetDevice(ctx->device), "set device");
  VGT_TRY_HIP(hipStreamSynchronize(ctx->stream), "drain stream");
  ctx->stream = ctx->own_stream;
  return VGT_HIP_OK;
}

int vgt_hip_synchronize(vgt_hip_ctx* ctx)
{
  if (!ctx) return Fail(VGT_HIP_ERR_INVALID_ARGUMENT, "null argument");
  VGT_TRY_HIP(hipSetDevice(ctx->device), "set device");
  VGT_TRY_HIP(hipStreamSynchronize(ctx->stream), "synchronize");
  {
    std::lock_guard<std::mutex> lock(ctx->mutex);
    if (ctx->copy_in) VGT_TRY_HIP(hipStreamSynchronize(ctx->copy_in), "synchronize the copy stream");
  }
  return VGT_HIP_OK;
}

int vgt_hip_device_of(const vgt_hip_ctx* ctx) { return ctx ? ctx->device : -1; }

#ifdef VGT_HIP_TESTING
int vgt_hip_set_edt_variant(vgt_hip_ctx* ctx, int variant)
{
  if (!ctx || variant < 0 || variant > 1) return Fail(VGT_HIP_ERR_INVALID_ARGUMENT, "invalid EDT variant");
  ctx->variant = variant;
  return VGT_HIP_OK;
}

int vgt_hip_debug_finalize_check(vgt_hip_ctx* ctx, int64_t first_d2, int64_t count, double resolution,
                                 uint64_t* mismatches, uint64_t* first_mismatch)
{
  if (!ctx || !mismatches || !first_mismatch || first_d2 < 0 || count <= 0 ||
      first_d2 + count > (int64_t{1} << 31))
    return Fail(VGT_HIP_ERR_INVALID_ARGUMENT, "invalid finalize-check range");
  VGT_TRY_HIP(hipSetDevice(ctx->device), "set device");
  unsigned long long host[2] = {0ull, ~0ull};
  vgt::HostStaging staging;
  const auto result = staging.InOut(host, 2);
  const int rc = staging.Run(*ctx, "finalize check", FailHip, [&](hipStream_t s) {
    return HipResult("finalize check", vgt::LaunchFinalizeCheck(first_d2, count, resolution, result.dev(), s));
  });
  if (rc != VGT_HIP_OK) return rc;
  *mismatches = host[0];
  *first_mismatch = host[1];
  return VGT_HIP_OK;
}

int vgt_hip_testing_set_host_pipeline_min_voxels(int64_t min_voxels)
{
  g_host_pipeline_min_voxels.store(min_voxels);
  return VGT_HIP_OK;
}

int vgt_hip_testing_set_short_line_rows(int rows)
{
  g_short_line_override.store(rows < 0 ? -1 : (rows > vgt::kShortLineRowsFewItems ? vgt::kShortLineRowsFewItems : rows));
  return VGT_HIP_OK;
}

int vgt_hip_testing_set_check_spheres_workgroups(int workgroups)
{
  g_check_spheres_workgroups.store(workgroups > 0 ? workgroups : 0);
  return VGT_HIP_OK;
}

int vgt_hip_testing_set_sphere_volume_workgroups(int workgroups)
{
  g_sphere_volume_workgroups.store(workgroups > 0 ? workgroups : 0);
  return VGT_HIP_OK;
}

int vgt_hip_testing_set_align_workgroups(int workgroups)
{
  g_align_workgroups.store(workgroups > 0 ? workgroups : 0);
  return VGT_HIP_OK;
}

int vgt_hip_testing_set_kinematics_workgroups(int workgroups)
{
  g_kinematics_workgroups.store(workgroups > 0 ? workgroups : 0);
  return VGT_HIP_OK;
}

int vgt_hip_testing_set_motion_workgroups(int workgroups)
{
  g_motion_workgroups.store(workgroups > 0 ? workgroups : 0);
  return VGT_HIP_OK;
}

int vgt_hip_testing_set_cost_workgroups(int workgroups)
{
  g_cost_workgroups.store(workgroups > 0 ? workgroups : 0);
  return VGT_HIP_OK;
}

int vgt_hip_testing_motion_launch_geometry(int64_t num_links, int64_t num_spheres, int32_t* tile_samples,
                                           int32_t* table_in_lds)
{
  if (!tile_samples || !table_in_lds) return Fail(VGT_HIP_ERR_INVALID_ARGUMENT, "null argument");
  if (num_spheres < 0) return Fail(VGT_HIP_ERR_INVALID_ARGUMENT, "negative sphere count");
  const vgt::MotionLaunchGeometry geometry = vgt::SelectMotionGeometry(num_links, num_spheres);
  if (geometry.tile <= 0) return Fail(VGT_HIP_ERR_INVALID_ARGUMENT, "a tree the motion kernel does not take");
  *tile_samples = geometry.tile;
  *table_in_lds = geometry.table_in_lds;
  return VGT_HIP_OK;
}

int vgt_hip_testing_cost_launch_geometry(int64_t num_links, int64_t num_spheres, int gradient_form, int32_t* tile_samples,
                                         int32_t* passes, int32_t* table_in_lds, int32_t* links_in_lds)
{
  if (!tile_samples || !passes || !table_in_lds || !links_in_lds)
    return Fail(VGT_HIP_ERR_INVALID_ARGUMENT, "null argument");
  if (num_spheres < 0) return Fail(VGT_HIP_ERR_INVALID_ARGUMENT, "negative sphere count");
  const vgt::CostLaunchGeometry geometry = vgt::SelectCostGeometry(num_links, num_spheres, gradient_form != 0);
  if (geometry.tile <= 0) return Fail(VGT_HIP_ERR_INVALID_ARGUMENT, "a tree the cost kernel does not take");
  *tile_samples = geometry.tile;
  *passes = geometry.passes;
  *table_in_lds = geometry.table_in_lds;
  *links_in_lds = geometry.links_in_lds;
  return VGT_HIP_OK;
}

int vgt_hip_testing_set_self_collision_workgroups(int workgroups)
{
  g_self_collision_workgroups.store(workgroups > 0 ? workgroups : 0);
  return VGT_HIP_OK;
}

int vgt_hip_testing_set_motion_self_workgroups(int workgroups)
{
  g_motion_self_workgroups.store(workgroups > 0 ? workgroups : 0);
  return VGT_HIP_OK;
}

int vgt_hip_testing_set_sphere_volume_counters(uint64_t* counters_dev)
{
  g_sphere_volume_counters.store(reinterpret_cast<unsigned long long*>(counters_dev));
  return VGT_HIP_OK;
}
// ... 4349 lines not shown
```

voxelized_geometry_tools_amd/csrc/vgt_internal.hpp:

```cpp
#pragma once

#include <hip/hip_runtime.h>

#include <cstddef>
#include <cstdint>

#include <string>

namespace vgt
{
void SetLastError(const std::string& message);
}
struct vgt_hip_ctx;
namespace vgt
{
hipStream_t ContextStream(const vgt_hip_ctx* ctx);

constexpr int16_t kInf16 = 32767;
constexpr int32_t kInf32 = 0x7fffffff;
constexpr int64_t kMaxExtent = 16384;

struct SdfParams
{
  int64_t nx, ny, nz;
  double resolution;
  int unknown_is_filled;
  int add_virtual_border;
  int64_t z_offset = 0;
  int64_t nz_global = 0;
  int64_t batch = 1;
};

struct ClassRecord
{
  uint32_t mask_lo, mask_hi, below2, above2;
};
constexpr uint32_t kRecordBias = 1u << 17;
constexpr uint32_t kRecordNoneBelow = 0u;
constexpr uint32_t kRecordNoneAbove = 2u * kRecordBias;
constexpr uint32_t kRecordNoSite = 0xfffffff0u;
inline int64_t RecordWords(int64_t nz) { return (nz + 63) / 64; }
constexpr int kRecordPadding = 256;
inline size_t ClassRecordBytes(int64_t nx, int64_t ny, int64_t nz)
{
  return (static_cast<size_t>(nx) * static_cast<size_t>(RecordWords(nz)) * static_cast<size_t>(ny) + kRecordPadding) *
         sizeof(ClassRecord);
}

struct SlabLineSummary
{
  uint16_t first, last;
};
constexpr uint16_t kSlabFilledBit = 0x8000u;
constexpr uint16_t kSlabNone = 0x7fffu;
inline void SlabRange(int64_t nz, int world, int rank, int64_t* z0, int64_t* count)
{
  const int64_t share = nz / world, extra = nz % world;
  *z0 = rank * share + (rank < extra ? rank : extra);
  *count = share + (rank < extra ? 1 : 0);
}
struct SlabLineCarry
{
  int16_t prev_filled, next_filled, prev_free, next_free;
};


hipError_t LaunchSlabCarries(const SlabLineSummary* summaries, int world, int rank, int64_t lines, int64_t nz_global,
                             SlabLineCarry* carries, hipStream_t stream);
hipError_t LaunchClassRecordsFromOccupancy(const float* occupancy, ClassRecord* records, const SdfParams& p,
                                           SlabLineSummary* summary, hipStream_t stream);
hipError_t LaunchClassRecordsFromMask(const uint8_t* mask, ClassRecord* records, const SdfParams& p,
                                      SlabLineSummary* summary, hipStream_t stream);
hipError_t LaunchSlabRecordFixup(ClassRecord* records, const SlabLineCarry* carries, const SdfParams& p,
                                 hipStream_t stream);
struct SweepScratch
{
  void* ptr;
  size_t bytes;
};
hipError_t LaunchPassYSweepRecords(const ClassRecord* records, int32_t* out32, SweepScratch scratch, const SdfParams& p,
                                   hipStream_t stream);
hipError_t LaunchPassXFinalize(const int32_t* in32, float* sdf, uint32_t* minmax_enc, SweepScratch scratch,
                               const SdfParams& p, hipStream_t stream);
constexpr int kShortLineRows = 64;
constexpr int kShortLineRowsFewItems = 128;
constexpr int64_t kFewLineItems = 1024;
int ShortLineOverride();
inline int ShortLineRows()
{
  const int told = ShortLineOverride();
  return told >= 0 ? told : kShortLineRows;
}
inline int ShortLineLimit(int64_t items)
{
  const int told = ShortLineOverride();
  if (told >= 0) return told;
  return items <= kFewLineItems ? kShortLineRowsFewItems : kShortLineRows;
}
hipError_t LaunchPassYShortRecords(const ClassRecord* records, int32_t* out32, const SdfParams& p, hipStream_t stream);
hipError_t LaunchPassXShortFinalizeRange(const int32_t* in32, float* sdf, uint32_t* minmax_enc, const SdfParams& p,
                                         int64_t outer_begin, int64_t outer_count, hipStream_t stream);
hipError_t LaunchPassXFinalizeRange(const int32_t* in32, float* sdf, uint32_t* minmax_enc, SweepScratch scratch,
                                    const SdfParams& p, int64_t outer_begin, int64_t outer_count, hipStream_t stream);
hipError_t LaunchPassXSweepFinalizeRange(const int32_t* in32, float* sdf, uint32_t* minmax_enc, SweepScratch scratch,
                                         const SdfParams& p, int64_t outer_begin, int64_t outer_count_or_all,
                                         hipStream_t stream);
hipError_t LaunchPassXSweepFinalize(const int32_t* in32, float* sdf, uint32_t* minmax_enc, SweepScratch scratch,
                                    const SdfParams& p, hipStream_t stream);
size_t SweepPassScratchBytes(int64_t nx, int64_t ny, int64_t nz, int64_t batch = 1);
hipError_t LaunchInitMinMax(uint32_t* minmax_enc, hipStream_t stream, int64_t count = 1);
hipError_t LaunchDecodeMinMax(const uint32_t* minmax_enc, float* minmax_out, hipStream_t stream, int64_t count = 1);

hipError_t LaunchCellMask(const void* cells_dev, int64_t num_cells, int cell_bytes, int object_id_offset,
                          int mode, const uint32_t* objects_dev, int num_objects, int unknown_is_filled,
                          uint8_t* mask_dev, hipStream_t stream);
hipError_t LaunchCellObjectMasks(const void* cells_dev, int64_t num_cells, int cell_bytes, int object_id_offset,
                                 const uint32_t* ids_dev, int num_ids, int unknown_is_filled, uint8_t* masks_dev,
                                 hipStream_t stream);
hipError_t LaunchDistinctObjectIds(const void* cells_dev, int64_t num_cells, int cell_bytes, int object_id_offset,
                                   uint32_t* table_dev, int table_log2, uint32_t* ids_dev, uint32_t* count_overflow_dev,
                                   hipStream_t stream);
hipError_t LaunchNextObjectId(const void* cells_dev, int64_t num_cells, int cell_bytes, int object_id_offset,
                              uint32_t after, uint32_t* result_dev, hipStream_t stream);
hipError_t LaunchCombineFreeAndNamed(const float* free_sdf_dev, const float* named_sdf_dev, int64_t num_cells,
                                     float* out_dev, uint32_t* minmax_enc, hipStream_t stream);

hipError_t LaunchCoarseGradient(const float* sdf_dev, int64_t nx, int64_t ny, int64_t nz, double resolution,
                                int enable_edge_gradients, const double* rotation_host, double* gradient_dev,
                                uint8_t* has_value_dev, hipStream_t stream);

hipError_t LaunchEstimateDistance(const float* sdf_dev, int64_t nx, int64_t ny, int64_t nz, double resolution,
                                  const double* grid_from_world_host, const double* queries_dev, int64_t num_queries,
                                  double* distance_dev, uint8_t* has_value_dev, hipStream_t stream);
hipError_t LaunchFineGradient(const float* sdf_dev, int64_t nx, int64_t ny, int64_t nz, double resolution,
                              const double* grid_from_world_host, const double* queries_dev, int64_t num_queries,
                              double nominal_window_size, double* gradient_dev, uint8_t* has_value_dev,
                              uint32_t* window_too_large_dev, hipStream_t stream);

int32_t DefaultProjectionIterations(int64_t nx, int64_t ny, int64_t nz, double stepsize_multiplier);
hipError_t LaunchProjectOutOfCollision(const float* sdf_dev, int64_t nx, int64_t ny, int64_t nz, double resolution,
                                       const double* grid_from_world_host, const double* rotation_host,
                                       const double* queries_dev, int64_t num_queries, double minimum_distance,
                                       double stepsize_multiplier, int32_t max_iterations, double* position_dev,
                                       uint8_t* has_value_dev, uint8_t* status_dev, int32_t* iterations_dev,
                                       hipStream_t stream);

size_t LocalExtremaScratchBytes(int64_t num_cells);
hipError_t LaunchLocalExtremaMap(const float* sdf_dev, int64_t nx, int64_t ny, int64_t nz, double resolution,
                                 const double* rotation_host, double* extrema_dev, void* scratch_dev,
                                 hipStream_t stream);

constexpr int kComponentClasses = 0;
constexpr int kComponentClassesAndIds = 1;
constexpr int kComponentSegments = 2;
constexpr int kComponentFill = 3;
size_t ComponentScratchBytes(int64_t num_cells);
const uint32_t* ComponentCountPtr(const void* scratch_dev, int64_t num_cells);
hipError_t LaunchLabelComponents(const void* cells_dev, int cell_bytes, int object_id_offset, int mode,
                                 const double* extrema_dev, double connected_threshold, int64_t nx, int64_t ny,
                                 int64_t nz, uint32_t* labels_dev, void* scratch_dev, hipStream_t stream);
size_t FillScratchBytes(int64_t num_cells);
const unsigned long long* FillCountPtr(const void* scratch_dev);
hipError_t LaunchFillEnclosed(void* cells_dev, int cell_bytes, int unknown_is_filled, int64_t nx, int64_t ny, int64_t nz,
                              void* scratch_dev, hipStream_t stream);
hipError_t LaunchComponentSurfaceMask(const float* occupancy_dev, const uint32_t* labels_dev, int64_t nx, int64_t ny,
                                      int64_t nz, int component_types, uint8_t* mask_dev, hipStream_t stream);

hipError_t LaunchScanBlocks(int32_t* block_counts_dev, int64_t blocks, uint32_t* total_dev, hipStream_t stream);

constexpr int kSelectAll = 0;
// ... 380 lines not shown
```

Before: 252,000 Mvoxels/s.

## Add coarse-hull X pass chosen on device from sampled one-class line counts

Adds a variant of the final X-pass sweep that first builds the lower envelope from a subsample of rows taken every 32 entries, spills it to a dedicated scratch region, then refines from it. The record kernel counts lines that hold only one class in a hashed subset of blocks. At launch, both plain and coarse kernels are enqueued and each reads the counts on device, so only the one matching the scene's one-class share does the work. This avoids full ring refills for suitable scenes, at the cost of extra atomics in the record pass, an extra near-empty kernel launch, and more spill scratch.

```diff
diff --git a/include/vgt_hip.h b/include/vgt_hip.h
--- a/include/vgt_hip.h
+++ b/include/vgt_hip.h
@@ -133,6 +133,12 @@
                                  uint64_t* first_mismatch);
 int vgt_hip_testing_set_host_pipeline_min_voxels(int64_t min_voxels);
 int vgt_hip_testing_set_short_line_rows(int rows);
+int vgt_hip_testing_one_class_counts(vgt_hip_ctx* ctx, const void* workspace_dev, int64_t nx, int64_t ny, int64_t nz,
+                                     uint32_t* counts);
+int vgt_hip_testing_set_sweep_slots(int slots);
+int vgt_hip_testing_set_coarse_hull(int mode);
+int vgt_hip_testing_x_pass_choice(vgt_hip_ctx* ctx, const void* workspace_dev, int64_t nx, int64_t ny, int64_t nz,
+                                  int32_t* choice);
 int vgt_hip_testing_set_check_spheres_workgroups(int workgroups);
 int vgt_hip_testing_set_sphere_volume_workgroups(int workgroups);
 int vgt_hip_testing_set_align_workgroups(int workgroups);
diff --git a/voxelized_geometry_tools_amd/capi.py b/voxelized_geometry_tools_amd/capi.py
--- a/voxelized_geometry_tools_amd/capi.py
+++ b/voxelized_geometry_tools_amd/capi.py
@@ -210,6 +210,10 @@
     "vgt_hip_debug_finalize_check": (_int, [_p, ctypes.c_int64, ctypes.c_int64, ctypes.c_double, _p, _p]),
     "vgt_hip_testing_set_host_pipeline_min_voxels": (_int, [ctypes.c_int64]),
     "vgt_hip_testing_set_short_line_rows": (_int, [_int]),
+    "vgt_hip_testing_set_coarse_hull": (_int, [_int]),
+    "vgt_hip_testing_set_sweep_slots": (_int, [_int]),
+    "vgt_hip_testing_one_class_counts": (_int, [_p, _p, _i64, _i64, _i64, _p]),
+    "vgt_hip_testing_x_pass_choice": (_int, [_p, _p, _i64, _i64, _i64, _p]),
     "vgt_hip_testing_set_check_spheres_workgroups": (_int, [_int]),
     "vgt_hip_testing_set_sphere_volume_workgroups": (_int, [_int]),
     "vgt_hip_testing_set_align_workgroups": (_int, [_int]),
@@ -1406,6 +1410,24 @@
     def set_short_line_rows(self, rows):
         check(self._lib.vgt_hip_testing_set_short_line_rows(int(rows)))
 
+    def one_class_counts(self, workspace_ptr, shape):
+        counts = (ctypes.c_uint32 * 2)()
+        check(self._lib.vgt_hip_testing_one_class_counts(self.handle, _ptr(workspace_ptr), *[int(v) for v in shape],
+                                                         ctypes.cast(counts, ctypes.c_void_p)))
+        return int(counts[0]), int(counts[1])
+
+    def set_sweep_slots(self, slots):
+        check(self._lib.vgt_hip_testing_set_sweep_slots(int(slots)))
+
+    def set_coarse_hull(self, mode):
+        check(self._lib.vgt_hip_testing_set_coarse_hull(int(mode)))
+
+    def x_pass_choice(self, workspace_ptr, shape):
+        choice = ctypes.c_int32(-1)
+        check(self._lib.vgt_hip_testing_x_pass_choice(self.handle, _ptr(workspace_ptr), *[int(v) for v in shape],
+                                                      ctypes.byref(choice)))
+        return int(choice.value)
+
     def set_check_spheres_workgroups(self, workgroups):
         check(self._lib.vgt_hip_testing_set_check_spheres_workgroups(int(workgroups)))
 
diff --git a/voxelized_geometry_tools_amd/csrc/edt_kernels.hip b/voxelized_geometry_tools_amd/csrc/edt_kernels.hip
--- a/voxelized_geometry_tools_amd/csrc/edt_kernels.hip
+++ b/voxelized_geometry_tools_amd/csrc/edt_kernels.hip
@@ -48,6 +48,7 @@
     minmax_enc[2 * i] = 0xffffffffu;
     minmax_enc[2 * i + 1] = 0u;
   }
+  if (count == 1 && threadIdx.x == 0) minmax_enc[kOneClassWord] = minmax_enc[kOneClassWord + 1] = 0u;
 }
 __global__ void DecodeMinMaxKernel(const uint32_t* minmax_enc, float* out, int count)
 {
diff --git a/voxelized_geometry_tools_amd/csrc/edt_line_geom.hpp b/voxelized_geometry_tools_amd/csrc/edt_line_geom.hpp
--- a/voxelized_geometry_tools_amd/csrc/edt_line_geom.hpp
+++ b/voxelized_geometry_tools_amd/csrc/edt_line_geom.hpp
@@ -14,6 +14,7 @@
   int groups;
   int nwords;
   int chunks;
+  int by_scene;
   int64_t row_stride;
   int64_t outer_stride;
   int nx, ny;
diff --git a/voxelized_geometry_tools_amd/csrc/edt_record_kernels.hip b/voxelized_geometry_tools_amd/csrc/edt_record_kernels.hip
--- a/voxelized_geometry_tools_amd/csrc/edt_record_kernels.hip
+++ b/voxelized_geometry_tools_amd/csrc/edt_record_kernels.hip
@@ -11,6 +11,7 @@
 constexpr int kRecordWaves = kRecordBlock / kWaveSize;
 constexpr int kNoTransitionBelow = -(1 << 20);
 constexpr int kNoTransitionAbove = 1 << 20;
+__device__ __forceinline__ bool CountsOneClassLines(uint32_t block) { return ((block * 0x9E3779B1u) >> 27) == 0u; }
 
 template <bool kUnknownFilled>
 __device__ __forceinline__ bool IsFilledCell(float occupancy)
@@ -48,9 +49,17 @@
                                                                  ClassRecord* __restrict__ records,
                                                                  int64_t num_lines, int ny, int nz, int nwords,
                                                                  SlabLineSummary* __restrict__ summary, int z_offset,
-                                                                 int mark_no_site)
+                                                                 int mark_no_site, uint32_t* __restrict__ one_class_lines)
 {
   constexpr int L = kWaveSize / W;
+  __shared__ uint32_t block_one_class, block_lines;
+  uint32_t wave_one_class = 0, wave_lines = 0;
+  if (one_class_lines && !CountsOneClassLines(blockIdx.x)) one_class_lines = nullptr;
+  if (one_class_lines)
+  {
+    if (threadIdx.x == 0) block_one_class = block_lines = 0u;
+    __syncthreads();
+  }
   const int lane = threadIdx.x & (kWaveSize - 1);
   const int wave = __builtin_amdgcn_readfirstlane(static_cast<int>(threadIdx.x) / kWaveSize);
   const int j = lane / W, w = lane % W;
@@ -118,6 +127,12 @@
     if (boundary) above = word_begin + 63;
     const int line_last = __shfl(upto, W - 1, W);
     const int line_first = __shfl(from, 0, W);
+    if (one_class_lines)
+    {
+      wave_one_class += static_cast<uint32_t>(__builtin_popcountll(__builtin_amdgcn_ballot_w64(
+          valid && w == 0 && mark_no_site && line_last == kNoTransitionBelow)));
+      wave_lines += static_cast<uint32_t>(lines_here);
+    }
     if (valid)
     {
       const uint32_t line = static_cast<uint32_t>(line0) + static_cast<uint32_t>(j);
@@ -156,6 +171,20 @@
       }
     }
   }
+  if (one_class_lines)
+  {
+    if (lane == 0)
+    {
+      atomicAdd(&block_one_class, wave_one_class);
+      atomicAdd(&block_lines, wave_lines);
+    }
+    __syncthreads();
+    if (threadIdx.x == 0)
+    {
+      if (block_one_class != 0u) atomicAdd(one_class_lines, block_one_class);
+      atomicAdd(one_class_lines + 1, block_lines);
+    }
+  }
 }
 
 template <typename InT, bool kUnknownFilled>
@@ -163,8 +192,17 @@
                                                                          ClassRecord* __restrict__ records,
                                                                          int64_t num_lines, int ny, int nz, int nwords,
                                                                          SlabLineSummary* __restrict__ summary,
-                                                                         int z_offset, int mark_no_site)
-{
+                                                                         int z_offset, int mark_no_site,
+                                                                         uint32_t* __restrict__ one_class_lines)
+{
+  __shared__ uint32_t block_one_class, block_lines;
+  uint32_t wave_one_class = 0, wave_lines = 0;
+  if (one_class_lines && !CountsOneClassLines(blockIdx.x)) one_class_lines = nullptr;
+  if (one_class_lines)
+  {
+    if (threadIdx.x == 0) block_one_class = block_lines = 0u;
+    __syncthreads();
+  }
   constexpr int kMaxWords = static_cast<int>(kMaxExtent / kWaveSize);
   __shared__ uint64_t s_mask[kRecordWaves][kMaxWords];
   __shared__ int32_t s_below[kRecordWaves][kMaxWords];
@@ -214,6 +252,8 @@
     const int64_t x = line / ny;
     const int y = static_cast<int>(line - x * ny);
     const int line_first = ends[0], line_last = ends[1];
+    if (mark_no_site && line_last == kNoTransitionBelow) wave_one_class++;
+    wave_lines++;
     for (int c = lane; c < nwords; c += kWaveSize)
     {
       const uint64_t m = mask[c];
@@ -235,6 +275,20 @@
       summary[line] = s;
     }
     __builtin_amdgcn_wave_barrier();
+  }
+  if (one_class_lines)
+  {
+    if (lane == 0)
+    {
+      atomicAdd(&block_one_class, wave_one_class);
+      atomicAdd(&block_lines, wave_lines);
+    }
+    __syncthreads();
+    if (threadIdx.x == 0)
+    {
+      if (block_one_class != 0u) atomicAdd(one_class_lines, block_one_class);
+      atomicAdd(one_class_lines + 1, block_lines);
+    }
   }
 }
 
@@ -303,10 +357,11 @@
   const int nwords = static_cast<int>(RecordWords(p.nz));
   const int z_offset = static_cast<int>(p.z_offset);
   const int mark_no_site = summary == nullptr ? 1 : 0;
+  uint32_t* const one_class_lines = p.one_class_lines;
 #define VGT_RECORD_CASE(W)                                                                                          \
   hipLaunchKernelGGL((ClassRecordKernel<InT, W, kUnknownFilled>), dim3(RecordGridFor((lines + 64 / W - 1) / (64 / W))), \
                      dim3(kRecordBlock), 0, stream, in, records, lines, ny, nz, nwords, summary, z_offset,          \
-                     mark_no_site)
+                     mark_no_site, one_class_lines)
   if (nwords <= 1)
     VGT_RECORD_CASE(1);
   else if (nwords <= 2)
@@ -323,7 +378,7 @@
     VGT_RECORD_CASE(64);
   else
     hipLaunchKernelGGL((ClassRecordLongLineKernel<InT, kUnknownFilled>), dim3(RecordGridFor(lines)), dim3(kRecordBlock),
-                       0, stream, in, records, lines, ny, nz, nwords, summary, z_offset, mark_no_site);
+                       0, stream, in, records, lines, ny, nz, nwords, summary, z_offset, mark_no_site, one_class_lines);
 #undef VGT_RECORD_CASE
   return hipGetLastError();
 }
diff --git a/voxelized_geometry_tools_amd/csrc/edt_sweep_kernels.hip b/voxelized_geometry_tools_amd/csrc/edt_sweep_kernels.hip
--- a/voxelized_geometry_tools_amd/csrc/edt_sweep_kernels.hip
+++ b/voxelized_geometry_tools_amd/csrc/edt_sweep_kernels.hip
@@ -3,6 +3,9 @@
 
 #include <cstdlib>
 #include <type_traits>
+#ifdef VGT_HOST_EMULATION
+#include <vector>
+#endif
 
 namespace vgt
 {
@@ -42,6 +45,18 @@
 constexpr int kSweepGroups = VGT_SWEEP_GROUPS;
 constexpr int kCounterStride = 32;
 constexpr int kMaxSweepSlots = 4096;
+constexpr int kCoarseStride = 32;
+constexpr int kCoarseShortest = 2 * kCoarseStride + 1;
+#ifdef VGT_HOST_EMULATION
+constexpr int kCoarseMinRows = kCoarseShortest;
+constexpr int kCoarseMinRounds = 0;
+#else
+constexpr int kCoarseMinRows = 512;
+constexpr int kCoarseMinRounds = 2;
+#endif
+constexpr uint32_t kCoarseShareLow = 18, kCoarseShareHigh = 27, kCoarseShareDen = 32;
+__host__ __device__ constexpr int CoarseChunks(int n) { return (n / kCoarseStride + 1 + 4 + 7) / 8 + 1; }
+constexpr int kChoiceWord = 1;
 template <bool kPacked>
 struct RingShape
 {
@@ -49,6 +64,7 @@
   static constexpr int kChunk = kPacked ? VGT_SWEEP_CHUNK : VGT_SWEEP_CHUNK_WIDE;
   static_assert(kBand % kChunk == 0 && kRing >= 4 * kChunk && (kRing & (kRing - 1)) == 0 && kChunk % 4 == 0, "sizes");
 };
+constexpr bool kCoarseBuilt = RingShape<true>::kChunk == 8;
 constexpr int kFar = 32768;
 static_assert(kWord % kBand == 0 && kBand % 2 == 0, "sizes");
 #ifdef VGT_HOST_EMULATION
@@ -56,6 +72,11 @@
 uint64_t ring_checks = 0, ring_spills = 0;
 constexpr uint32_t kInfoPoison = 0xdeadbeefu;
 uint64_t sign_word_reads = 0;
+struct CoarseDrop
+{
+  int item, lane, row;
+};
+std::vector<CoarseDrop> coarse_dropped;
 #endif
 
 
@@ -331,7 +352,7 @@
 #endif
 }
 
-template <typename InT, typename OutT, bool kFinal, bool kPacked, bool kPlain>
+template <typename InT, typename OutT, bool kFinal, bool kPacked, bool kPlain, bool kCoarse = false>
 __global__ __launch_bounds__(kWaveSize, VGT_SWEEP_WAVES) void SweepPassKernel(const InT* __restrict__ in,
                                                                             OutT* __restrict__ out,
                                                                             unsigned char* __restrict__ spill,
@@ -346,6 +367,19 @@
   constexpr bool kSignBlocks = !kFinal;
   constexpr bool kTakeSignWords = !kSignBlocks;
   static_assert(!(kRecords && kFinal), "records feed the Y pass");
+  static_assert(!kCoarse || (kFinal && kPacked && kPlain), "the coarse hull is built for the plain X pass with 32-bit entries");
+  if constexpr (kFinal && kPacked && kPlain)
+  {
+    if (g.by_scene)
+    {
+      const uint32_t one_class = __builtin_amdgcn_readfirstlane(minmax_enc[kOneClassWord]) * kCoarseShareDen;
+      const uint32_t counted = __builtin_amdgcn_readfirstlane(minmax_enc[kOneClassWord + 1]);
+      const bool coarse_scene = static_cast<int>(one_class >= counted * kCoarseShareLow) &
+                                static_cast<int>(one_class < counted * kCoarseShareHigh);
+      if (coarse_scene != kCoarse) return;
+    }
+    if (blockIdx.x == 0 && threadIdx.x == 0) work_counter[kChoiceWord] = (kCoarse ? 2 : 1) + (g.by_scene ? 4 : 0);
+  }
   constexpr int kRing = RingShape<kPacked>::kRing;
   constexpr int kChunk = RingShape<kPacked>::kChunk;
   constexpr int32_t kLimit = C::kSentinelG;
@@ -363,6 +397,8 @@
   const int64_t rstride = g.row_stride;
   unsigned char* const own_spill = spill + static_cast<int64_t>(blockIdx.x) * g.chunks * (kWaveSize * kChunkBytes);
   uint2* const own_info = word_info + static_cast<int64_t>(blockIdx.x) * (g.nwords + 1) * kWaveSize;
+  [[maybe_unused]] unsigned char* const own_coarse =
+      kCoarse ? own_spill + static_cast<int64_t>(g.chunks - CoarseChunks(g.n)) * (kWaveSize * kChunkBytes) : nullptr;
   const uint32_t lane_entry = static_cast<uint32_t>(lane) * kEntryBytes;
   const uint32_t lane_chunk = static_cast<uint32_t>(lane) * kChunkBytes;
   float lo_value = INFINITY, hi_value = -INFINITY;
@@ -494,9 +530,9 @@
   {
     auto check_ring = [&]() {
       const uint32_t resident = D - L;
-      const bool refilling = static_cast<int>(pf_count != 0) |
-                             (static_cast<int>(L != 0) & static_cast<int>(resident <= kChunkSlots));
-      if (__builtin_expect(__builtin_amdgcn_ballot_w64(refilling) != 0ull, 0))
+      const bool refilling = !kCoarse && (static_cast<int>(pf_count != 0) |
+                                          (static_cast<int>(L != 0) & static_cast<int>(resident <= kChunkSlots)));
+      if (!kCoarse && __builtin_expect(__builtin_amdgcn_ballot_w64(refilling) != 0ull, 0))
       {
         VGT_COLD_PATH();
         if (pf_count != 0)
@@ -732,17 +768,130 @@
         }
       };
       int32_t nxt[kBand];
-      load_band(nxt, 0);
+      if constexpr (!kCoarse) load_band(nxt, 0);
       constexpr int32_t kNoSiteG = 0x60000000;
       auto decode = [&](int32_t v, int q, int32_t& G) {
         const int32_t f = static_cast<int32_t>(min(static_cast<uint32_t>(v) & 0x7fffffffu, static_cast<uint32_t>(kNoSiteG)));
         G = f + q * q;
       };
+      [[maybe_unused]] Entry chb = C::Unknown(), chc = C::Unknown();
+      [[maybe_unused]] int32_t low_G = 0;
+      [[maybe_unused]] int low_row = -1, ch_next = 0;
+      [[maybe_unused]] auto coarse_entry = [&](int index) -> Entry {
+        const uint32_t chunk_first = static_cast<uint32_t>(index / kChunk) * kChunkSlots;
+        return reinterpret_cast<const Entry*>(own_coarse + (chunk_first + lane_chunk))[index % kChunk];
+      };
+      if constexpr (kCoarse)
+      {
+        static_assert(kCoarseStride % kBand == 0, "a band never holds two vertices of the subsample's hull");
+        static_assert(kChunk == 8, "CoarseChunks counts chunks of eight entries");
+        wave_spill = own_coarse;
+        constexpr int kBatch = 2 * kBand;
+        for (int s0 = 0; s0 < n; s0 += kBatch * kCoarseStride)
+        {
+          int32_t sub[kBatch];
+          {
+            const int last_sub = (n - 1) / kCoarseStride * kCoarseStride;
+#pragma unroll
+            for (int k = 0; k < kBatch; k++)
+            {
+              const int q = min(s0 + k * kCoarseStride, last_sub);
+              const VGT_GLOBAL InT* row_in = UniformPointer(GlobalPointer(wave_in + static_cast<int64_t>(q) * rstride));
+              sub[k] = static_cast<int32_t>(*LaneAddress(row_in, lane_bytes));
+            }
+          }
+#pragma unroll
+          for (int k = 0; k < kBatch; k++)
+          {
+            const int q = s0 + k * kCoarseStride;
+            if (q < n)
+            {
+              if (k % kChunk == 0) check_ring();
+              int32_t G_sub;
+              decode(sub[k], q, G_sub);
+              site(q, G_sub, true);
+            }
+          }
+        }
+        const bool in_ring = L == 0u;
+        for (uint32_t first = L; __builtin_amdgcn_ballot_w64(first <= D) != 0ull;)
+        {
+          if (first <= D)
+          {
+            Entry buf[kChunk];
+            Entry* const slots = chunk_in_ring(first);
+#pragma unroll
+            for (int j = 0; j < kChunk; j++)
+            {
+              buf[j] = chunk_slot(slots, first, j);
+              if (first + (static_cast<uint32_t>(j) << kShift) >= D) buf[j] = C::Unknown();
+            }
+            StoreChunk(spill_ptr(first), buf);
+            first += kChunkSlots;
+          }
+        }
+        if (in_ring)
+        {
+          if (D > (4u << kShift)) chb = ring_ref(4u << kShift);
+          if (D > (5u << kShift)) chc = ring_ref(5u << kShift);
+        }
+        ch_next = 5;
+        if (__builtin_expect(__builtin_amdgcn_ballot_w64(!in_ring) != 0ull, 0))
+        {
+          VGT_COLD_PATH();
+          if (!in_ring)
+          {
+            chb = coarse_entry(4);
+            if (!C::IsUnknown(chb)) chc = coarse_entry(5);
+          }
+        }
+        wave_spill = own_spill;
+        D = 4u << kShift;
+        L = 0;
+        Gt = C::kSentinelG;
+        nB = 1;
+        rt = 0;
+        A = 0;
+        e3 = C::Pack(C::kSentinelG + 2, 0);
+        pf_count = 0;
+        ring_ref(0u << kShift) = C::Pack(0, 0);
+        ring_ref(1u << kShift) = C::Pack(C::kSentinelG + 2, 0);
+        ring_ref(2u << kShift) = C::Pack(C::kSentinelG + 1, 0);
+        ring_ref(3u << kShift) = C::Pack(C::kSentinelG, 0);
+        load_band(nxt, 0);
+      }
       int32_t G_prev = kNoSiteG, G_cur = 0;
       decode(nxt[0], 0, G_cur);
       for (int r0 = 0; r0 < n; r0 += kBand)
       {
         __builtin_assume(r0 >= 0 && r0 < 16384);
+        [[maybe_unused]] int32_t chord_G = 0, chord_dG = 0;
+        [[maybe_unused]] int chord_row = 0, chord_width = 0;
+        if constexpr (kCoarse)
+        {
+          const bool arrived = static_cast<int>(!C::IsUnknown(chb)) & static_cast<int>(r0 >= C::Row(chb));
+          if (__builtin_amdgcn_ballot_w64(arrived) != 0ull)
+          {
+            if (arrived)
+            {
+              low_G = C::G(chb);
+              low_row = C::Row(chb);
+              chb = chc;
+              if (!C::IsUnknown(chc))
+              {
+                ch_next++;
+                chc = coarse_entry(ch_next);
+              }
+            }
+          }
+          chord_G = low_G;
+          chord_row = low_row;
+          if (static_cast<int>(low_row >= 0) & static_cast<int>(!C::IsUnknown(chb)))
+          {
+            chord_dG = C::G(chb) - low_G;
+            chord_width = C::Row(chb) - low_row;
+          }
+        }
         int32_t cur[kBand];
 #pragma unroll
         for (int k = 0; k < kBand; k++) cur[k] = nxt[k];
@@ -769,7 +918,17 @@
               bits = __builtin_amdgcn_alignbit(bits, static_cast<uint32_t>(cur[k]), 31);
               int32_t G_next = kNoSiteG + (q + 1) * (q + 1);
               if ((!kGuard && k + 1 < kBand) || q + 1 < n) decode(k + 1 < kBand ? cur[k + 1] : nxt[0], q + 1, G_next);
-              site(q, G_cur, G_cur - G_prev < G_next - G_cur);
+              if constexpr (kCoarse)
+              {
+                const bool above = static_cast<int64_t>(G_cur - chord_G) * chord_width -
+                                       static_cast<int64_t>(chord_dG) * (q - chord_row) > 0;
+#ifdef VGT_HOST_EMULATION
+                if (above && G_cur < kNoSiteG) coarse_dropped.push_back(CoarseDrop{item, lane, q});
+#endif
+                site(q, G_cur, static_cast<int>(G_cur - G_prev < G_next - G_cur) & static_cast<int>(!above));
+              }
+              else
+                site(q, G_cur, G_cur - G_prev < G_next - G_cur);
               G_prev = G_cur;
               G_cur = G_next;
             }
@@ -1244,10 +1403,16 @@
   return n <= 1024 && max_input + (n - 1) * (n - 1) < Codec<true>::kSentinelG;
 }
 
+int64_t CoarseAreaChunks(int64_t n, bool packed)
+{
+  return (kCoarseBuilt && packed && n >= kCoarseShortest) ? CoarseChunks(static_cast<int>(n)) : 0;
+}
+
 size_t SlotScratchBytes(int64_t n, bool packed)
 {
   const int64_t nwords = (n + kWord - 1) / kWord;
-  const size_t spill = packed ? SpillChunks(n, RingShape<true>::kChunk) * kWaveSize * RingShape<true>::kChunk * sizeof(uint32_t)
+  const size_t spill = packed ? (SpillChunks(n, RingShape<true>::kChunk) + CoarseAreaChunks(n, packed)) * kWaveSize *
+                                    RingShape<true>::kChunk * sizeof(uint32_t)
                               : SpillChunks(n, RingShape<false>::kChunk) * kWaveSize * RingShape<false>::kChunk * sizeof(uint2);
   return spill + static_cast<size_t>(nwords + 1) * kWaveSize * sizeof(uint2);
 }
@@ -1262,7 +1427,7 @@
 
 template <typename InT, typename OutT, bool kFinal>
 hipError_t LaunchSweep(const InT* in, OutT* out, void* scratch, size_t scratch_bytes, uint32_t* minmax_enc, SweepGeom g,
-                       int64_t outer_count, int64_t max_input, hipStream_t stream)
+                       int64_t outer_count, int64_t max_input, hipStream_t stream, int x_kernel = kXKernelPlain)
 {
   g.zsegs = (g.nz + kWaveSize - 1) / kWaveSize;
   g.nwords = (g.n + kWord - 1) / kWord;
@@ -1278,6 +1443,9 @@
   }
   const bool packed = PackedEntries(g.n, max_input);
   int64_t slots = items < kSweepSlots ? items : kSweepSlots;
+#ifndef VGT_HOST_EMULATION
+  if (const int told = SweepSlotsOverride(); told > 0 && told < slots) slots = told;
+#endif
   {
     const size_t per_slot = SlotScratchBytes(g.n, packed);
     const int64_t fit = scratch_bytes > kCounterBytes ? static_cast<int64_t>((scratch_bytes - kCounterBytes) / per_slot) : 0;
@@ -1287,6 +1455,11 @@
   g.groups = static_cast<int>(slots < kSweepGroups ? slots : kSweepGroups);
   const int chunk = packed ? RingShape<true>::kChunk : RingShape<false>::kChunk;
   g.chunks = static_cast<int>(SpillChunks(g.n, chunk));
+  const bool general = kFinal && (g.add_virtual_border || !(g.resolution > 1.0e-30 && g.resolution < 1.0e30));
+  bool coarse = kFinal && kCoarseBuilt && x_kernel != kXKernelPlain && packed && !general && g.batch_outers == g.outers && g.n >= kCoarseShortest;
+  if (x_kernel == kXKernelByScene) coarse = coarse && g.n >= kCoarseMinRows && items >= kCoarseMinRounds * slots;
+  if (coarse) g.chunks += CoarseChunks(g.n);
+  if (coarse && x_kernel == kXKernelByScene) g.by_scene = 1;
   char* bytes = static_cast<char*>(scratch);
   int* counter = reinterpret_cast<int*>(bytes);
   unsigned char* spill = reinterpret_cast<unsigned char*>(bytes + kCounterBytes);
@@ -1297,7 +1470,6 @@
   *counter = 0;
 #endif
   const dim3 grid(static_cast<unsigned>(slots)), block(kWaveSize);
-  const bool general = kFinal && (g.add_virtual_border || !(g.resolution > 1.0e-30 && g.resolution < 1.0e30));
 #ifndef VGT_HOST_EMULATION
   {
     const hipError_t err = hipMemsetAsync(counter, 0, kSweepGroups * kCounterStride * sizeof(int), stream);
@@ -1307,6 +1479,16 @@
 #define VGT_LAUNCH_SWEEP(PACKED, PLAIN)                                                                             \
   hipLaunchKernelGGL((SweepPassKernel<InT, OutT, kFinal, PACKED, PLAIN>), grid, block, 0, stream, in, out, spill, info, \
                      minmax_enc, counter, g)
+  if constexpr (kFinal && kCoarseBuilt)
+  {
+    if (coarse)
+    {
+      if (g.by_scene) VGT_LAUNCH_SWEEP(true, true);
+      hipLaunchKernelGGL((SweepPassKernel<InT, OutT, true, true, true, true>), grid, block, 0, stream, in, out, spill, info,
+                         minmax_enc, counter, g);
+      return hipGetLastError();
+    }
+  }
   if (packed && general)
     VGT_LAUNCH_SWEEP(true, !kFinal);
   else if (packed)
@@ -1368,8 +1550,11 @@
     g.outer_begin = static_cast<int>(outer_begin);
     outer_count = outer_count_or_all;
   }
+  int x_kernel = p.x_kernel;
+  if (outer_count_or_all >= 0 || p.batch > 1) x_kernel = kXKernelPlain;
+  if (x_kernel == kXKernelByScene && p.one_class_lines != minmax_enc + kOneClassWord) x_kernel = kXKernelPlain;
   return LaunchSweep<int32_t, float, true>(in32, sdf, scratch.ptr, scratch.bytes, minmax_enc, g, outer_count,
-                                           MaxInputX(p), stream);
+                                           MaxInputX(p), stream, x_kernel);
 }
 
 hipError_t LaunchPassXSweepFinalize(const int32_t* in32, float* sdf, uint32_t* minmax_enc, SweepScratch scratch,
diff --git a/voxelized_geometry_tools_amd/csrc/vgt_hip_capi.hip b/voxelized_geometry_tools_amd/csrc/vgt_hip_capi.hip
--- a/voxelized_geometry_tools_amd/csrc/vgt_hip_capi.hip
+++ b/voxelized_geometry_tools_amd/csrc/vgt_hip_capi.hip
@@ -130,6 +130,8 @@
 {
 thread_local std::string g_last_error;
 std::atomic<int> g_short_line_override{-1};
+std::atomic<int> g_sweep_slots_override{0};
+std::atomic<int> g_coarse_hull_mode{vgt::kXKernelByScene};
 std::atomic<int> g_check_spheres_workgroups{0};
 std::atomic<int> g_align_workgroups{0};
 std::atomic<int> g_kinematics_workgroups{0};
@@ -152,6 +154,7 @@
 void SetLastError(const std::string& message) { g_last_error = message; }
 hipStream_t ContextStream(const vgt_hip_ctx* ctx) { return ctx->stream; }
 int ShortLineOverride() { return g_short_line_override.load(); }
+int SweepSlotsOverride() { return g_sweep_slots_override.load(); }
 }
 namespace
 {
@@ -392,6 +395,15 @@
   }
   return vgt::LaunchPassYSweepRecords(ws.records + first_slice * vgt::RecordWords(part.nz) * part.ny,
                                       ws.t32 + voxel_offset, ws.sweep_scratch, part, s);
+}
+vgt::SdfParams WithKernelByScene(const SdfWorkspace& ws, vgt::SdfParams p)
+{
+  if (p.batch == 1 && ws.records)
+  {
+    p.one_class_lines = ws.minmax_enc + vgt::kOneClassWord;
+    p.x_kernel = g_coarse_hull_mode.load();
+  }
+  return p;
 }
 hipError_t LaunchPassThree(const SdfWorkspace& ws, const vgt::SdfParams& p, float* sdf_dev, hipStream_t s)
 {
@@ -730,16 +742,17 @@
 }
 
 template <typename InT>
-int RunSdfPipeline(vgt_hip_ctx* ctx, const InT* input_dev, const vgt::SdfParams& p, float* sdf_dev,
+int RunSdfPipeline(vgt_hip_ctx* ctx, const InT* input_dev, const vgt::SdfParams& given, float* sdf_dev,
                    void* workspace_dev, size_t workspace_bytes, float* minmax_dev,
                    hipEvent_t* events)
 {
-  if (p.batch > 1 && ctx->variant != 0)
+  if (given.batch > 1 && ctx->variant != 0)
     return Fail(VGT_HIP_ERR_INVALID_ARGUMENT, "batches run on the default EDT pipeline only");
-  const SdfWorkspace ws = CarveWorkspace(workspace_dev, p.nx, p.ny, p.nz, ctx->variant, p.batch);
+  const SdfWorkspace ws = CarveWorkspace(workspace_dev, given.nx, given.ny, given.nz, ctx->variant, given.batch);
   if (workspace_dev == nullptr || workspace_bytes < ws.bytes)
     return Fail(VGT_HIP_ERR_INVALID_ARGUMENT, "SDF workspace too small");
   hipStream_t s = ctx->stream;
+  const vgt::SdfParams p = WithKernelByScene(ws, given);
   vgt::SdfParams slices = p;
   slices.nx = p.nx * p.batch;
   slices.batch = 1;
@@ -1476,6 +1489,50 @@
 int vgt_hip_testing_set_short_line_rows(int rows)
 {
   g_short_line_override.store(rows < 0 ? -1 : (rows > vgt::kShortLineRowsFewItems ? vgt::kShortLineRowsFewItems : rows));
+  return VGT_HIP_OK;
+}
+
+int vgt_hip_testing_set_sweep_slots(int slots)
+{
+  g_sweep_slots_override.store(slots > 0 ? slots : 0);
+  return VGT_HIP_OK;
+}
+
+int vgt_hip_testing_set_coarse_hull(int mode)
+{
+  if (mode != vgt::kXKernelByScene && mode != vgt::kXKernelCoarse && mode != vgt::kXKernelPlain)
+    return Fail(VGT_HIP_ERR_INVALID_ARGUMENT, "coarse-hull mode must be 0 (by scene), 1 (always) or 2 (never)");
+  g_coarse_hull_mode.store(mode);
+  return VGT_HIP_OK;
+}
+
+int vgt_hip_testing_x_pass_choice(vgt_hip_ctx* ctx, const void* workspace_dev, int64_t nx, int64_t ny, int64_t nz,
+                                  int32_t* choice)
+{
+  if (!ctx || !workspace_dev || !choice) return Fail(VGT_HIP_ERR_INVALID_ARGUMENT, "null argument");
+  const int rc = CheckSdfShape(nx, ny, nz, 1.0);
+  if (rc != VGT_HIP_OK) return rc;
+  VGT_TRY_HIP(hipSetDevice(ctx->device), "set device");
+  const SdfWorkspace ws = CarveWorkspace(const_cast<void*>(workspace_dev), nx, ny, nz, ctx->variant);
+  std::lock_guard<std::mutex> lock(ctx->mutex);
+  VGT_TRY_HIP(hipStreamSynchronize(ctx->stream), "synchronize");
+  VGT_TRY_HIP(hipMemcpy(choice, static_cast<const char*>(ws.sweep_scratch.ptr) + sizeof(int32_t), sizeof(int32_t),
+                        hipMemcpyDeviceToHost),
+              "copy");
+  return VGT_HIP_OK;
+}
+
+int vgt_hip_testing_one_class_counts(vgt_hip_ctx* ctx, const void* workspace_dev, int64_t nx, int64_t ny, int64_t nz,
+                                     uint32_t* counts)
+{
+  if (!ctx || !workspace_dev || !counts) return Fail(VGT_HIP_ERR_INVALID_ARGUMENT, "null argument");
+  const int rc = CheckSdfShape(nx, ny, nz, 1.0);
+  if (rc != VGT_HIP_OK) return rc;
+  VGT_TRY_HIP(hipSetDevice(ctx->device), "set device");
+  const SdfWorkspace ws = CarveWorkspace(const_cast<void*>(workspace_dev), nx, ny, nz, ctx->variant);
+  std::lock_guard<std::mutex> lock(ctx->mutex);
+  VGT_TRY_HIP(hipStreamSynchronize(ctx->stream), "synchronize");
+  VGT_TRY_HIP(hipMemcpy(counts, ws.minmax_enc + vgt::kOneClassWord, 2 * sizeof(uint32_t), hipMemcpyDeviceToHost), "copy");
   return VGT_HIP_OK;
 }
 
diff --git a/voxelized_geometry_tools_amd/csrc/vgt_internal.hpp b/voxelized_geometry_tools_amd/csrc/vgt_internal.hpp
--- a/voxelized_geometry_tools_amd/csrc/vgt_internal.hpp
+++ b/voxelized_geometry_tools_amd/csrc/vgt_internal.hpp
@@ -20,6 +20,7 @@
 constexpr int32_t kInf32 = 0x7fffffff;
 constexpr int64_t kMaxExtent = 16384;
 
+constexpr int kXKernelByScene = 0, kXKernelCoarse = 1, kXKernelPlain = 2;
 struct SdfParams
 {
   int64_t nx, ny, nz;
@@ -29,7 +30,10 @@
   int64_t z_offset = 0;
   int64_t nz_global = 0;
   int64_t batch = 1;
-};
+  uint32_t* one_class_lines = nullptr;
+  int x_kernel = kXKernelPlain;
+};
+constexpr int kOneClassWord = 2;
 
 struct ClassRecord
 {
@@ -86,6 +90,7 @@
 constexpr int kShortLineRowsFewItems = 128;
 constexpr int64_t kFewLineItems = 1024;
 int ShortLineOverride();
+int SweepSlotsOverride();
 inline int ShortLineRows()
 {
   const int told = ShortLineOverride();
```

New measurement: 257,400 Mvoxels/s (median of 6 runs). +2.2%, better.
